# LLNL/parelagmc

Measured on AMD Instinct MI355X. Metric: MC samples/sec (SPDE field + Darcy QoI) at stated DoF; SpMV HBM GB/s vs roofline, higher is better.
Workload: dtype f64; 1 GPU; PDESampler cube_tet r=5, 595968 DoF (n_s=196608, n_u=399360, nnz(A)=4299072), 1 MC level, corlen 0.1, SPDE field only (BASELINE config 2), 4 x 64 realizations per step, all converged; tolerance=MINRES 300 / rel 1e-6 / abs 1e-12, solver=hybridization, batch=64, streams=4, parallelism=sample-farm x1, precond_storage=fp32

## Files before the change

include/pmc.h:

```cpp
#ifndef PMC_H_
#define PMC_H_

#include <stddef.h>
#include <stdint.h>

#ifdef __cplusplus
extern "C" {
#endif

#define PMC_OK 0
#define PMC_ERR_INVALID (-1)
#define PMC_ERR_DEVICE (-2)
#define PMC_ERR_COMM (-3)
#define PMC_ERR_INTERNAL (-4)

enum pmc_memspace { PMC_MEM_HOST = 0, PMC_MEM_DEVICE = 1 };
enum pmc_projection { PMC_PROJ_NONE = 0, PMC_PROJ_GATHER = 1, PMC_PROJ_L2 = 2 };
enum pmc_storage { PMC_STORAGE_FP32 = 0, PMC_STORAGE_FP64 = 1 };

typedef struct pmc_ctx pmc_ctx;
typedef struct pmc_sampler pmc_sampler;
typedef struct pmc_darcy pmc_darcy;

typedef struct pmc_csr {
// ... 3 lines not shown
    const double* vals;
} pmc_csr;

typedef struct pmc_solver_opts {
    int32_t abi_version;
    int32_t max_iter;
    double rel_tol;
    double abs_tol;
    int32_t cheb_degree_M;
    double cheb_ratio_M;
    int32_t mg_smooth_degree;
    double mg_smooth_ratio;
    int32_t mg_coarse_degree;
    double mg_coarse_ratio;
    int32_t check_every;
    int32_t use_graph;
    double schur_scale;
    int32_t mg_coarsening;
    int32_t mini_max_rows;
    int32_t two_streams;
    int32_t precond_storage;
} pmc_solver_opts;

typedef struct pmc_stats {
    int32_t iterations;
    int32_t converged;
    double initial_norm;
    double final_norm;
    double solve_ms;
    double setup_ms;
} pmc_stats;

typedef struct pmc_sampler_level {
    int32_t n_u, n_s;
    pmc_csr M;
    pmc_csr B;
    const double* w_diag;
    pmc_csr P;
} pmc_sampler_level;

typedef struct pmc_hybrid_level {
    int32_t n_lambda, n_s;
    pmc_csr H;
    pmc_csr G;
    const double* z_diag;
    const double* w_diag;
    pmc_csr P;
} pmc_hybrid_level;

typedef struct pmc_hybrid_elements {
    int32_t n_u, n_s;
    pmc_csr M_pattern;
    const int32_t* c_ptr;
    const int32_t* c_elem;
    const double* c_val;
    pmc_csr B;
    const double* w_diag;
    pmc_csr P;
} pmc_hybrid_elements;
typedef struct pmc_hybrid_system pmc_hybrid_system;

typedef struct pmc_darcy_level {
    int32_t n_u, n_p;
    pmc_csr M_pattern;
    const int32_t* c_ptr;
    const int32_t* c_elem;
    const double* c_val;
    pmc_csr B;
    const double* rhs;
    const uint8_t* ess_mask;
    const double* ess_data;
    const double* obs;
    pmc_csr P;
} pmc_darcy_level;

int pmc_version(void);
#define PMC_ABI_VERSION 3
int pmc_abi_version(void);
int pmc_krylov_z_bytes(void);
int pmc_sampler_krylov_z_bytes(const pmc_sampler* s);
int pmc_darcy_krylov_z_bytes(const pmc_darcy* d);
uint64_t pmc_kernel_launches(void);
uint64_t pmc_fused_lanczos_solves(void);
const char* pmc_last_error(void);
void pmc_solver_opts_default(pmc_solver_opts* opts);

int pmc_ctx_create(int device_id, pmc_ctx** out);
int pmc_ctx_create_abi(int device_id, int abi_version, pmc_ctx** out);
#ifndef PMC_NO_ABI_CHECK_MACRO
#define pmc_ctx_create(device_id, out) pmc_ctx_create_abi((device_id), PMC_ABI_VERSION, (out))
#endif
void pmc_ctx_destroy(pmc_ctx* ctx);
int pmc_ctx_synchronize(pmc_ctx* ctx);
void* pmc_ctx_stream(pmc_ctx* ctx);
int pmc_ctx_device(const pmc_ctx* ctx);
int pmc_timer_start(pmc_ctx* ctx);
int pmc_timer_stop(pmc_ctx* ctx, double* ms);

int pmc_malloc(pmc_ctx* ctx, size_t bytes, void** dptr);
int pmc_free(pmc_ctx* ctx, void* dptr);
int pmc_memcpy_h2d(pmc_ctx* ctx, void* dst, const void* src, size_t bytes);
int pmc_memcpy_d2h(pmc_ctx* ctx, void* dst, const void* src, size_t bytes);

int pmc_rng_seed(pmc_ctx* ctx, uint64_t seed, int nparts, int mypart);
int pmc_normal_fill(pmc_ctx* ctx, double mean, double sigma2, uint64_t first_sample_id, uint32_t stream,
                    int nbatch, int n, double* out, int memspace);

int pmc_sampler_create(pmc_ctx* ctx, int nlevels, int n_mc_levels, const pmc_sampler_level* levels,
                       double alpha, double matern_g, int lognormal, const pmc_solver_opts* opts,
                       pmc_sampler** out);
int pmc_sampler_create_hybrid(pmc_ctx* ctx, int nlevels, const pmc_hybrid_level* levels, double alpha, double matern_g,
                              int lognormal, const pmc_solver_opts* opts, pmc_sampler** out);
int pmc_sampler_is_hybrid(const pmc_sampler* s);
int pmc_hybrid_build(const pmc_hybrid_elements* level, double alpha, pmc_hybrid_system** out);
int pmc_hybrid_system_level(const pmc_hybrid_system* sys, pmc_hybrid_level* view);
void pmc_hybrid_system_destroy(pmc_hybrid_system* sys);
int pmc_sampler_create_hybrid_from_elements(pmc_ctx* ctx, int nlevels, const pmc_hybrid_elements* levels, double alpha,
                                            double matern_g, int lognormal, const pmc_solver_opts* opts, pmc_sampler** out);
typedef struct pmc_kl_level {
    int32_t n_s;
    const double* w_diag;
    pmc_csr P;
} pmc_kl_level;
int pmc_sampler_create_kl(pmc_ctx* ctx, int nlevels, const pmc_kl_level* levels, int nmodes, const double* evals,
                          const double* evect0, int lognormal, pmc_sampler** out);
int pmc_sampler_is_kl(const pmc_sampler* s);
typedef struct pmc_kl_eigs_opts {
    double tol;
    int32_t max_iter;
    int32_t guard;
    int32_t degree;
    uint64_t seed;
} pmc_kl_eigs_opts;
typedef struct pmc_kl_eigs_info {
    int32_t iterations;
    int32_t block_products;
    int32_t converged;
    double max_residual_rel;
    double gap_rel;
    double seconds;
} pmc_kl_eigs_info;
void pmc_kl_eigs_opts_default(pmc_kl_eigs_opts* opts);
int pmc_kl_matern_apply(pmc_ctx* ctx, int dim, int n, const double* centroids, const double* w_diag, double corlen,
                        int ncols, const double* X, double* Y);
int pmc_kl_matern_eigs(pmc_ctx* ctx, int dim, int n, const double* centroids, const double* w_diag, double corlen,
                       int nmodes, const pmc_kl_eigs_opts* opts , double* evals ,
                       double* evect0 , pmc_kl_eigs_info* info );
void pmc_sampler_destroy(pmc_sampler* s);
int pmc_sampler_set_projection(pmc_sampler* s, int level, int kind, const pmc_csr* Gt,
                               const int32_t* gather_idx, const double* inv_w_orig, int orig_size);
int pmc_sampler_num_levels(const pmc_sampler* s);
int pmc_sampler_xi_size(const pmc_sampler* s, int level);
int pmc_sampler_sample_size(const pmc_sampler* s, int level);
int64_t pmc_sampler_nnz(const pmc_sampler* s, int level);
int pmc_sampler_batch_width(const pmc_sampler* s, int level);
int pmc_sampler_true_p(const pmc_sampler* s, int level, pmc_csr* out);
int pmc_sampler_sample(pmc_sampler* s, int level, uint64_t first_sample_id, int nbatch, double* xi,
                       int memspace);
int pmc_sampler_eval(pmc_sampler* s, int level, int xi_level, int nbatch, const double* xi, double* s_out,
                     const double* init_s, int init_level, int use_init, double* embed_s_out, int memspace,
                     pmc_stats* stats);

typedef struct pmc_field_stats pmc_field_stats;
int pmc_field_stats_create(pmc_sampler* s, int level, const double* chi, int memspace, pmc_field_stats** out);
void pmc_field_stats_destroy(pmc_field_stats* fs);
int pmc_field_stats_reset(pmc_field_stats* fs);
// ... 95 lines not shown
```

parelagmc_amd/capi.py:

```python
from __future__ import annotations

import ctypes as C
import weakref
import os
from typing import Optional, Sequence

import numpy as np

_HERE = os.path.dirname(os.path.abspath(__file__))
LIB_PATH = os.path.join(_HERE, "lib", "libpmc.so")

PMC_MEM_HOST, PMC_MEM_DEVICE = 0, 1
PMC_PROJ_NONE, PMC_PROJ_GATHER, PMC_PROJ_L2 = 0, 1, 2


class PmcError(RuntimeError):
    def __init__(self, code, msg):
        super().__init__(f"libpmc error {code}: {msg}")
        self.code = code


class pmc_csr(C.Structure):
    _fields_ = [("nrows", C.c_int32), ("ncols", C.c_int32), ("rowptr", C.POINTER(C.c_int32)),
                ("colind", C.POINTER(C.c_int32)), ("vals", C.POINTER(C.c_double))]


class pmc_solver_opts(C.Structure):
    _fields_ = [("abi_version", C.c_int32), ("max_iter", C.c_int32), ("rel_tol", C.c_double), ("abs_tol", C.c_double),
                ("cheb_degree_M", C.c_int32), ("cheb_ratio_M", C.c_double),
                ("mg_smooth_degree", C.c_int32), ("mg_smooth_ratio", C.c_double),
                ("mg_coarse_degree", C.c_int32), ("mg_coarse_ratio", C.c_double), ("check_every", C.c_int32),
                ("use_graph", C.c_int32), ("schur_scale", C.c_double), ("mg_coarsening", C.c_int32), ("mini_max_rows", C.c_int32),
                ("two_streams", C.c_int32), ("precond_storage", C.c_int32)]


PMC_ABI_VERSION = 3
PMC_STORAGE_FP32, PMC_STORAGE_FP64 = 0, 1


class pmc_stats(C.Structure):
    _fields_ = [("iterations", C.c_int32), ("converged", C.c_int32), ("initial_norm", C.c_double),
                ("final_norm", C.c_double), ("solve_ms", C.c_double), ("setup_ms", C.c_double)]


class pmc_sampler_level(C.Structure):
    _fields_ = [("n_u", C.c_int32), ("n_s", C.c_int32), ("M", pmc_csr), ("B", pmc_csr),
                ("w_diag", C.POINTER(C.c_double)), ("P", pmc_csr)]


class pmc_hybrid_level(C.Structure):
    _fields_ = [("n_lambda", C.c_int32), ("n_s", C.c_int32), ("H", pmc_csr), ("G", pmc_csr),
                ("z_diag", C.POINTER(C.c_double)), ("w_diag", C.POINTER(C.c_double)), ("P", pmc_csr)]


class pmc_hybrid_elements(C.Structure):
    _fields_ = [("n_u", C.c_int32), ("n_s", C.c_int32), ("M_pattern", pmc_csr), ("c_ptr", C.POINTER(C.c_int32)),
                ("c_elem", C.POINTER(C.c_int32)), ("c_val", C.POINTER(C.c_double)), ("B", pmc_csr),
                ("w_diag", C.POINTER(C.c_double)), ("P", pmc_csr)]


class pmc_kl_level(C.Structure):
    _fields_ = [("n_s", C.c_int32), ("w_diag", C.POINTER(C.c_double)), ("P", pmc_csr)]


class pmc_kl_eigs_opts(C.Structure):
    _fields_ = [("tol", C.c_double), ("max_iter", C.c_int32), ("guard", C.c_int32), ("degree", C.c_int32),
                ("seed", C.c_uint64)]


class pmc_kl_eigs_info(C.Structure):
    _fields_ = [("iterations", C.c_int32), ("block_products", C.c_int32), ("converged", C.c_int32),
                ("max_residual_rel", C.c_double), ("gap_rel", C.c_double), ("seconds", C.c_double)]


class pmc_darcy_level(C.Structure):
    _fields_ = [("n_u", C.c_int32), ("n_p", C.c_int32), ("M_pattern", pmc_csr), ("c_ptr", C.POINTER(C.c_int32)),
                ("c_elem", C.POINTER(C.c_int32)), ("c_val", C.POINTER(C.c_double)), ("B", pmc_csr),
                ("rhs", C.POINTER(C.c_double)), ("ess_mask", C.POINTER(C.c_uint8)),
                ("ess_data", C.POINTER(C.c_double)), ("obs", C.POINTER(C.c_double)), ("P", pmc_csr)]


_VP = C.c_void_p
_DP = C.c_void_p
SYMBOLS = {
    "pmc_version": (C.c_int, []),
    "pmc_last_error": (C.c_char_p, []),
    "pmc_solver_opts_default": (None, [C.POINTER(pmc_solver_opts)]),
    "pmc_abi_version": (C.c_int, []),
    "pmc_krylov_z_bytes": (C.c_int, []),
    "pmc_sampler_krylov_z_bytes": (C.c_int, [_VP]),
    "pmc_darcy_krylov_z_bytes": (C.c_int, [_VP]),
    "pmc_kernel_launches": (C.c_uint64, []),
    "pmc_fused_lanczos_solves": (C.c_uint64, []),
    "pmc_ctx_create": (C.c_int, [C.c_int, C.POINTER(_VP)]),
    "pmc_ctx_create_abi": (C.c_int, [C.c_int, C.c_int, C.POINTER(_VP)]),
    "pmc_ctx_destroy": (None, [_VP]),
    "pmc_ctx_synchronize": (C.c_int, [_VP]),
    "pmc_ctx_stream": (_VP, [_VP]),
    "pmc_ctx_device": (C.c_int, [_VP]),
    "pmc_timer_start": (C.c_int, [_VP]),
    "pmc_timer_stop": (C.c_int, [_VP, C.POINTER(C.c_double)]),
    "pmc_malloc": (C.c_int, [_VP, C.c_size_t, C.POINTER(_VP)]),
    "pmc_free": (C.c_int, [_VP, _VP]),
    "pmc_memcpy_h2d": (C.c_int, [_VP, _VP, _VP, C.c_size_t]),
    "pmc_memcpy_d2h": (C.c_int, [_VP, _VP, _VP, C.c_size_t]),
    "pmc_rng_seed": (C.c_int, [_VP, C.c_uint64, C.c_int, C.c_int]),
    "pmc_normal_fill": (C.c_int, [_VP, C.c_double, C.c_double, C.c_uint64, C.c_uint32, C.c_int, C.c_int, _DP, C.c_int]),
    "pmc_sampler_create": (C.c_int, [_VP, C.c_int, C.c_int, C.POINTER(pmc_sampler_level), C.c_double, C.c_double,
                                     C.c_int, C.POINTER(pmc_solver_opts), C.POINTER(_VP)]),
    "pmc_sampler_create_hybrid": (C.c_int, [_VP, C.c_int, C.POINTER(pmc_hybrid_level), C.c_double, C.c_double, C.c_int,
                                            C.POINTER(pmc_solver_opts), C.POINTER(_VP)]),
    "pmc_sampler_is_hybrid": (C.c_int, [_VP]),
    "pmc_sampler_create_kl": (C.c_int, [_VP, C.c_int, C.POINTER(pmc_kl_level), C.c_int, C.POINTER(C.c_double),
                                        C.POINTER(C.c_double), C.c_int, C.POINTER(_VP)]),
    "pmc_sampler_is_kl": (C.c_int, [_VP]),
    "pmc_kl_eigs_opts_default": (None, [C.POINTER(pmc_kl_eigs_opts)]),
    "pmc_kl_matern_apply": (C.c_int, [_VP, C.c_int, C.c_int, C.POINTER(C.c_double), C.POINTER(C.c_double), C.c_double, C.c_int,
                                      C.POINTER(C.c_double), C.POINTER(C.c_double)]),
    "pmc_kl_matern_eigs": (C.c_int, [_VP, C.c_int, C.c_int, C.POINTER(C.c_double), C.POINTER(C.c_double), C.c_double, C.c_int,
                                     C.POINTER(pmc_kl_eigs_opts), C.POINTER(C.c_double), C.POINTER(C.c_double),
                                     C.POINTER(pmc_kl_eigs_info)]),
    "pmc_hybrid_build": (C.c_int, [C.POINTER(pmc_hybrid_elements), C.c_double, C.POINTER(_VP)]),
    "pmc_hybrid_system_level": (C.c_int, [_VP, C.POINTER(pmc_hybrid_level)]),
    "pmc_hybrid_system_destroy": (None, [_VP]),
    "pmc_sampler_create_hybrid_from_elements": (C.c_int, [_VP, C.c_int, C.POINTER(pmc_hybrid_elements), C.c_double, C.c_double,
                                                          C.c_int, C.POINTER(pmc_solver_opts), C.POINTER(_VP)]),
    "pmc_sampler_smoother_time": (C.c_int, [_VP, C.POINTER(C.c_double), C.POINTER(C.c_int64), C.POINTER(C.c_double)]),
    "pmc_sampler_smoother_bytes": (C.c_int, [_VP, C.c_int, C.c_int, C.POINTER(C.c_double)]),
    "pmc_sampler_vcycle_info": (C.c_int, [_VP, C.c_int, C.c_int, C.POINTER(C.c_int), C.POINTER(C.c_int64)]),
    "pmc_sampler_vcycle_level": (C.c_int, [_VP, C.c_int, C.c_int, C.POINTER(C.c_int), C.POINTER(C.c_double)]),
    "pmc_sampler_vcycle_prolongator": (C.c_int, [_VP, C.c_int, C.c_int, C.POINTER(C.c_int), C.POINTER(C.c_int),
                                                 C.POINTER(C.c_int64), C.POINTER(C.c_int32), C.POINTER(C.c_int32),
                                                 C.POINTER(C.c_double)]),
    "pmc_sampler_destroy": (None, [_VP]),
    "pmc_sampler_set_projection": (C.c_int, [_VP, C.c_int, C.c_int, C.POINTER(pmc_csr), C.POINTER(C.c_int32),
                                             C.POINTER(C.c_double), C.c_int]),
    "pmc_sampler_num_levels": (C.c_int, [_VP]),
    "pmc_sampler_xi_size": (C.c_int, [_VP, C.c_int]),
    "pmc_sampler_sample_size": (C.c_int, [_VP, C.c_int]),
    "pmc_sampler_batch_width": (C.c_int, [_VP, C.c_int]),
    "pmc_darcy_batch_width": (C.c_int, [_VP, C.c_int]),
    "pmc_darcy_set_operator_timing": (C.c_int, [_VP, C.c_int]),
    "pmc_darcy_operator_time": (C.c_int, [_VP, C.POINTER(C.c_double), C.POINTER(C.c_int64), C.POINTER(C.c_double)]),
    "pmc_darcy_operator_bytes": (C.c_int, [_VP, C.c_int, C.c_int, C.POINTER(C.c_double)]),
    "pmc_darcy_poly_time": (C.c_int, [_VP, C.POINTER(C.c_double), C.POINTER(C.c_int64), C.POINTER(C.c_double)]),
    "pmc_darcy_poly_bytes": (C.c_int, [_VP, C.c_int, C.c_int, C.POINTER(C.c_double)]),
    "pmc_sampler_nnz": (C.c_int64, [_VP, C.c_int]),
    "pmc_sampler_true_p": (C.c_int, [_VP, C.c_int, C.POINTER(pmc_csr)]),
    "pmc_sampler_sample": (C.c_int, [_VP, C.c_int, C.c_uint64, C.c_int, _DP, C.c_int]),
    "pmc_sampler_eval": (C.c_int, [_VP, C.c_int, C.c_int, C.c_int, _DP, _DP, _DP, C.c_int, C.c_int, _DP, C.c_int,
                                   C.POINTER(pmc_stats)]),
    "pmc_sampler_mult": (C.c_int, [_VP, C.c_int, C.c_int, _DP, _DP, C.c_int, C.c_int, C.POINTER(pmc_stats)]),
    "pmc_sampler_apply_preconditioner": (C.c_int, [_VP, C.c_int, C.c_int, _DP, _DP, C.c_int]),
    "pmc_sampler_apply_operator": (C.c_int, [_VP, C.c_int, C.c_int, _DP, _DP, C.c_int, C.c_int, C.POINTER(C.c_double),
                                             C.POINTER(C.c_double)]),
    "pmc_sampler_set_operator_timing": (C.c_int, [_VP, C.c_int]),
    "pmc_sampler_operator_time": (C.c_int, [_VP, C.POINTER(C.c_double), C.POINTER(C.c_int64)]),
    "pmc_sampler_operator_event_overhead": (C.c_int, [_VP, C.POINTER(C.c_double)]),
    "pmc_conditioner_create": (C.c_int, [_VP, C.c_int, C.POINTER(pmc_csr), C.POINTER(C.c_double), C.POINTER(C.c_double),
                                         C.POINTER(_VP)]),
    "pmc_conditioner_destroy": (None, [_VP]),
    "pmc_conditioner_num_obs": (C.c_int, [_VP]),
    "pmc_conditioner_level": (C.c_int, [_VP, C.c_int, C.POINTER(C.c_int), C.POINTER(C.c_int64), C.POINTER(C.c_double),
                                        C.POINTER(C.c_double), C.POINTER(C.c_int32), C.POINTER(C.c_int32),
                                        C.POINTER(C.c_double)]),
    "pmc_conditioner_apply": (C.c_int, [_VP, C.c_int, C.c_int, _DP, _DP, _DP, C.c_int, C.c_int]),
    "pmc_sampler_set_conditioner": (C.c_int, [_VP, _VP]),
    "pmc_field_stats_create": (C.c_int, [_VP, C.c_int, _DP, C.c_int, C.POINTER(_VP)]),
    "pmc_field_stats_destroy": (None, [_VP]),
    "pmc_field_stats_reset": (C.c_int, [_VP]),
    "pmc_field_stats_accumulate": (C.c_int, [_VP, C.c_int, _DP, C.c_int]),
    "pmc_field_stats_run": (C.c_int, [_VP, C.c_uint64, C.c_int64]),
    "pmc_field_stats_read": (C.c_int, [_VP, _DP, _DP, _DP, C.POINTER(C.c_int64), C.c_int]),
    "pmc_field_stats_read_sums": (C.c_int, [_VP, _DP, C.POINTER(C.c_int64), C.c_int]),
    "pmc_field_stats_chi_dot": (C.c_int, [_VP, C.c_int, _DP, _DP, C.c_int]),
    "pmc_sampler_l2_error": (C.c_int, [_VP, C.c_int, C.c_int, _DP, C.c_double, _DP, C.c_int]),
    "pmc_sampler_max_error": (C.c_int, [_VP, C.c_int, C.c_int, _DP, C.c_double, _DP, C.c_int]),
    "pmc_sampler_set_output_hierarchy": (C.c_int, [_VP, C.c_int, C.POINTER(pmc_csr), C.POINTER(C.c_double)]),
    "pmc_darcy_create": (C.c_int, [_VP, C.c_int, C.c_int, C.POINTER(pmc_darcy_level), C.c_int,
                                   C.POINTER(pmc_solver_opts), C.POINTER(_VP)]),
    "pmc_darcy_create_hybrid": (C.c_int, [_VP, C.c_int, C.c_int, C.POINTER(pmc_darcy_level), C.c_int,
                                          C.POINTER(pmc_solver_opts), C.POINTER(_VP)]),
    "pmc_darcy_destroy": (None, [_VP]),
    "pmc_darcy_num_dofs": (C.c_int, [_VP, C.c_int]),
    "pmc_darcy_num_pressure_dofs": (C.c_int, [_VP, C.c_int]),
    "pmc_darcy_nnz": (C.c_int64, [_VP, C.c_int]),
    "pmc_darcy_solve_fwd": (C.c_int, [_VP, C.c_int, C.c_int, _DP, C.POINTER(C.c_double), C.POINTER(C.c_double), _DP,
                                      C.c_int, C.POINTER(pmc_stats)]),
    "pmc_darcy_solve_fwd_pressure": (C.c_int, [_VP, C.c_int, C.c_int, _DP, _DP, C.POINTER(C.c_double),
                                               C.POINTER(C.c_double), C.c_int, C.c_int, C.POINTER(pmc_stats)]),
    "pmc_level_fields_create": (C.c_int, [_VP, _VP, C.c_int, C.c_int, C.POINTER(_VP)]),
    "pmc_level_fields_destroy": (None, [_VP]),
    "pmc_level_fields_reset": (C.c_int, [_VP]),
    "pmc_level_fields_accumulate": (C.c_int, [_VP, C.c_int, _DP, _DP, C.c_int]),
    "pmc_level_fields_accumulate_weighted": (C.c_int, [_VP, C.c_int, _DP, _DP, _DP, _DP, C.c_int]),
    "pmc_level_fields_read_sums": (C.c_int, [_VP, _DP, C.POINTER(C.c_int64), C.c_int]),
    "pmc_level_fields_size": (C.c_int, [_VP, C.POINTER(C.c_int), C.POINTER(C.c_int)]),
    "pmc_level_fields_parents": (C.c_int, [_VP, C.POINTER(C.c_int32)]),
    "pmc_darcy_apply_preconditioner": (C.c_int, [_VP, C.c_int, C.c_int, _DP, _DP, _DP, C.c_int]),
    "pmc_darcy_apply_operator": (C.c_int, [_VP, C.c_int, C.c_int, _DP, _DP, _DP, C.c_int]),
    "pmc_darcy_vcycle_level": (C.c_int, [_VP, C.c_int, C.c_int, C.POINTER(C.c_int), C.POINTER(C.c_double)]),
    "pmc_darcy_vcycle_prolongator": (C.c_int, [_VP, C.c_int, C.c_int, C.POINTER(C.c_int), C.POINTER(C.c_int),
                                               C.POINTER(C.c_int64), C.POINTER(C.c_int32), C.POINTER(C.c_int32),
                                               C.POINTER(C.c_double)]),
    "pmc_darcy_set_observations": (C.c_int, [_VP, C.c_int, C.POINTER(pmc_csr)]),
    "pmc_darcy_num_observations": (C.c_int, [_VP, C.c_int]),
    "pmc_darcy_compute_G": (C.c_int, [_VP, C.c_int, C.c_int, _DP, C.POINTER(C.c_double), C.POINTER(C.c_double),
                                      C.POINTER(C.c_double), C.c_int, C.POINTER(pmc_stats)]),
    "pmc_comm_unique_id": (C.c_int, [_VP]),
    "pmc_comm_init": (C.c_int, [_VP, _VP, C.c_int, C.c_int]),
    "pmc_comm_destroy": (C.c_int, [_VP]),
    "pmc_allreduce_sum_f64": (C.c_int, [_VP, C.POINTER(C.c_double), C.c_int]),
}

_lib = None


def load_library(path: Optional[str] = None):
    global _lib
    if _lib is not None and path is None:
        return _lib
    p = path or os.environ.get("PMC_LIB") or LIB_PATH
    if not os.path.exists(p):
        raise PmcError(-2, f"{p} not found - build it with `make` / __graft_entry__.build() (no CPU fallback)")
    lib = C.CDLL(p)
    for name, (res, args) in SYMBOLS.items():
        fn = getattr(lib, name)
        fn.restype = res
        fn.argtypes = args
    if path is None:
        _lib = lib
    return lib


def _check(rc):
    if rc != 0:
        raise PmcError(rc, load_library().pmc_last_error().decode("utf-8", "replace"))


def _i32(a):
    return np.ascontiguousarray(a, dtype=np.int32)


def _f64(a):
    return np.ascontiguousarray(a, dtype=np.float64)


def _ptr(a, ctype):
    return a.ctypes.data_as(C.POINTER(ctype))


class _Keep:

    def __init__(self):
        self.refs = []

    def csr(self, m) -> pmc_csr:
        if m is None:
            return pmc_csr(0, 0, None, None, None)
        m = m.tocsr()
        rp, ci, v = _i32(m.indptr), _i32(m.indices), _f64(m.data)
        self.refs += [rp, ci, v]
        return pmc_csr(m.shape[0], m.shape[1], _ptr(rp, C.c_int32), _ptr(ci, C.c_int32), _ptr(v, C.c_double))

    def f64(self, a):
        a = _f64(a)
        self.refs.append(a)
        return _ptr(a, C.c_double)

    def i32(self, a):
        a = _i32(a)
        self.refs.append(a)
        return _ptr(a, C.c_int32)

    def u8(self, a):
        a = np.ascontiguousarray(a, dtype=np.uint8)
        self.refs.append(a)
        return _ptr(a, C.c_uint8)


def hybrid_build(pattern, c_ptr, c_elem, c_val, B, w_diag, alpha, P=None):
    import scipy.sparse as sp
    lib = load_library()
    keep = _Keep()
    n_s, n_u = B.shape
    lv = pmc_hybrid_elements(n_u, n_s, keep.csr(pattern), keep.i32(c_ptr), keep.i32(c_elem), keep.f64(c_val), keep.csr(B),
                             keep.f64(w_diag), keep.csr(P))
    h = _VP()
    _check(lib.pmc_hybrid_build(C.byref(lv), float(alpha), C.byref(h)))
    try:
        v = pmc_hybrid_level()
        _check(lib.pmc_hybrid_system_level(h, C.byref(v)))

        def mat(c):
            rp = np.ctypeslib.as_array(c.rowptr, (c.nrows + 1,)).copy()
            nnz = int(rp[-1])
            return sp.csr_matrix((np.ctypeslib.as_array(c.vals, (nnz,)).copy(), np.ctypeslib.as_array(c.colind, (nnz,)).copy(), rp),
                                 shape=(c.nrows, c.ncols))
        return mat(v.H), mat(v.G), np.ctypeslib.as_array(v.z_diag, (n_s,)).copy()
    finally:
        lib.pmc_hybrid_system_destroy(h)


def library_hybrid_builder(space, alpha):
    from .fe.rt0 import mass_contributions
    pat, c_ptr, c_elem, c_val = mass_contributions(space.emass)
    return hybrid_build(pat, c_ptr, c_elem, c_val, space.B, space.vol, alpha)


# ... 828 lines not shown
```

parelagmc_amd/csrc/capi.hip:

```cpp
#include <dlfcn.h>

#include <atomic>
#include <cstdlib>
#include <cstring>
#include <mutex>

#include "handles.hpp"

namespace pmc {

static thread_local std::string g_last_error;
void set_last_error(const std::string& m) { g_last_error = m; }

void Ctx::activate() const { PMC_HIP(hipSetDevice(device)); }
void Ctx::phase_mark(int i) const { PMC_HIP(hipEventRecord(ev_phase[i], stream)); }
void Ctx::phase_report(pmc_stats* stats, int nb) const {
    PMC_HIP(hipEventSynchronize(ev_phase[2]));
    float setup = 0.f, solve = 0.f;
    PMC_HIP(hipEventElapsedTime(&setup, ev_phase[0], ev_phase[1]));
    PMC_HIP(hipEventElapsedTime(&solve, ev_phase[1], ev_phase[2]));
    for (int k = 0; k < nb; ++k) {
        stats[k].setup_ms = (double)setup / nb;
        stats[k].solve_ms = (double)solve / nb;
    }
}

static std::atomic<int> g_live_ctx[64];
int Ctx::contexts_on_device(int device) { return g_live_ctx[device & 63].load(); }

Lanes Ctx::lanes(bool split) {
    if (split && !stream2) {
        PMC_HIP(hipStreamCreateWithFlags(&stream2, hipStreamNonBlocking));
        PMC_HIP(hipEventCreateWithFlags(&ev_fork, hipEventDisableTiming));
        PMC_HIP(hipEventCreateWithFlags(&ev_join, hipEventDisableTiming));
    }
    return Lanes{stream, split ? stream2 : stream, ev_fork, ev_join, split};
}

template <class F>
static int guarded(F&& f) {
    try {
        f();
        return PMC_OK;
    } catch (const Error& e) {
        set_last_error(e.what());
        return e.code;
    } catch (const std::bad_alloc&) {
        set_last_error("host allocation failed");
        return PMC_ERR_INTERNAL;
    } catch (const std::exception& e) {
        set_last_error(e.what());
        return PMC_ERR_INTERNAL;
    } catch (...) {
        set_last_error("unknown exception");
        return PMC_ERR_INTERNAL;
    }
}

struct UniqueId { char internal[128]; };
struct Rccl {
    void* lib = nullptr;
    int (*GetUniqueId)(UniqueId*) = nullptr;
    int (*CommInitRank)(void**, int, UniqueId, int) = nullptr;
    int (*AllReduce)(const void*, void*, size_t, int, int, void*, hipStream_t) = nullptr;
    int (*CommDestroy)(void*) = nullptr;
    const char* (*GetErrorString)(int) = nullptr;
};
static Rccl& rccl() {
    static Rccl r;
    static std::once_flag once;
    std::call_once(once, [] {
        const char* names[] = {"librccl.so.1", "librccl.so", "/opt/rocm/lib/librccl.so.1", "/opt/rocm/lib/librccl.so"};
        for (const char* n : names) {
            r.lib = dlopen(n, RTLD_NOW | RTLD_LOCAL);
            if (r.lib) break;
        }
        if (!r.lib) return;
        r.GetUniqueId = reinterpret_cast<decltype(r.GetUniqueId)>(dlsym(r.lib, "ncclGetUniqueId"));
        r.CommInitRank = reinterpret_cast<decltype(r.CommInitRank)>(dlsym(r.lib, "ncclCommInitRank"));
        r.AllReduce = reinterpret_cast<decltype(r.AllReduce)>(dlsym(r.lib, "ncclAllReduce"));
        r.CommDestroy = reinterpret_cast<decltype(r.CommDestroy)>(dlsym(r.lib, "ncclCommDestroy"));
        r.GetErrorString = reinterpret_cast<decltype(r.GetErrorString)>(dlsym(r.lib, "ncclGetErrorString"));
    });
    if (!r.lib || !r.GetUniqueId || !r.CommInitRank || !r.AllReduce || !r.CommDestroy)
        throw Error(PMC_ERR_COMM, "RCCL (librccl.so) could not be loaded");
    return r;
}
static void rccl_check(int rc, const char* what) {
    if (rc != 0) {
        Rccl& r = rccl();
        throw Error(PMC_ERR_COMM, std::string(what) + ": " + (r.GetErrorString ? r.GetErrorString(rc) : "RCCL error"));
    }
}

}

using namespace pmc;

extern "C" {

int pmc_version(void) { return 100; }
int pmc_abi_version(void) { return PMC_ABI_VERSION; }
int pmc_krylov_z_bytes(void) { return 4; }
uint64_t pmc_kernel_launches(void) { return kernel_launch_count(); }
uint64_t pmc_fused_lanczos_solves(void) { return fused_lanczos_solve_count(); }
const char* pmc_last_error(void) { return g_last_error.c_str(); }

static void check_abi(const pmc_solver_opts& o) {
    if (o.abi_version != PMC_ABI_VERSION)
        throw Error(PMC_ERR_INVALID, "pmc_solver_opts.abi_version is " + std::to_string(o.abi_version) + ", this library has " +
                                         std::to_string(PMC_ABI_VERSION) +
                                         ": fill the struct with pmc_solver_opts_default() of the header you compile against");
}

void pmc_solver_opts_default(pmc_solver_opts* o) {
    if (!o) return;
    o->max_iter = 300;
    o->rel_tol = 1e-6;
    o->abs_tol = 1e-12;
    o->abi_version = PMC_ABI_VERSION;
    o->cheb_degree_M = 0;
    o->cheb_ratio_M = 0.0;
    o->mg_smooth_degree = 2;
    o->mg_smooth_ratio = 8.0;
    o->mg_coarse_degree = 12;
    o->mg_coarse_ratio = 100.0;
    o->check_every = 2;
    o->schur_scale = 1.0;
    o->mg_coarsening = 2;
    o->mini_max_rows = 6000;
    o->two_streams = 0;
    o->use_graph = 0;
    o->precond_storage = PMC_STORAGE_FP32;
}

#undef pmc_ctx_create
int pmc_ctx_create(int device_id, pmc_ctx** out);
int pmc_ctx_create_abi(int device_id, int abi_version, pmc_ctx** out) {
    if (abi_version != PMC_ABI_VERSION) {
        if (out) *out = nullptr;
        set_last_error("caller was compiled against PMC_ABI_VERSION " + std::to_string(abi_version) + ", this library has " +
                       std::to_string(PMC_ABI_VERSION) + " (layout of pmc_solver_opts / pmc_stats): rebuild against include/pmc.h");
        return PMC_ERR_INVALID;
    }
    return pmc_ctx_create(device_id, out);
}
int pmc_ctx_create(int device_id, pmc_ctx** out) {
    return guarded([&] {
        PMC_REQUIRE(out != nullptr, "pmc_ctx_create: out is NULL");
        *out = nullptr;
        int ndev = 0;
        hipError_t e = hipGetDeviceCount(&ndev);
        if (e != hipSuccess || ndev == 0)
            throw Error(PMC_ERR_DEVICE, "no HIP device available (libpmc has no CPU fallback)");
        PMC_REQUIRE(device_id >= 0 && device_id < ndev, "pmc_ctx_create: device id out of range");
        std::unique_ptr<pmc_ctx> c(new pmc_ctx());
        c->device = device_id;
        PMC_HIP(hipSetDevice(device_id));
        PMC_HIP(hipStreamCreateWithFlags(&c->stream, hipStreamNonBlocking));
        PMC_HIP(hipEventCreate(&c->ev0));
        PMC_HIP(hipEventCreate(&c->ev1));
        for (hipEvent_t& e : c->ev_phase) PMC_HIP(hipEventCreate(&e));
        PMC_HIP(hipHostMalloc(reinterpret_cast<void**>(&c->h_flag), sizeof(int) * 16, hipHostMallocDefault));
        PMC_HIP(hipHostMalloc(reinterpret_cast<void**>(&c->h_scal), sizeof(double) * pmc::Ctx::kHostScratch, hipHostMallocDefault));
        g_live_ctx[device_id & 63].fetch_add(1);
        *out = c.release();
    });
}

void pmc_ctx_destroy(pmc_ctx* c) {
    if (!c) return;
    g_live_ctx[c->device & 63].fetch_sub(1);
    (void)hipSetDevice(c->device);
    if (c->nccl) {
        try { rccl().CommDestroy(c->nccl); } catch (...) {}
        c->nccl = nullptr;
    }
    if (c->stream) (void)hipStreamSynchronize(c->stream);
    if (c->stream2) (void)hipStreamSynchronize(c->stream2);
    if (c->h_flag) (void)hipHostFree(c->h_flag);
    if (c->h_scal) (void)hipHostFree(c->h_scal);
    if (c->ev0) (void)hipEventDestroy(c->ev0);
    if (c->ev1) (void)hipEventDestroy(c->ev1);
    for (hipEvent_t e : c->ev_phase)
        if (e) (void)hipEventDestroy(e);
    for (hipEvent_t e : {c->ev_fork, c->ev_join})
        if (e) (void)hipEventDestroy(e);
    if (c->stream2) (void)hipStreamDestroy(c->stream2);
// ... 724 lines not shown
```

parelagmc_amd/csrc/handles.hpp:

```cpp
#pragma once
#include "solver.hpp"

namespace pmc {

HostCsr schur_host(const HostCsr& B, const HostCsr& Bt, const std::vector<double>& dM, const double* diag_add);
std::unique_ptr<Multigrid> build_sa_chain(const HostCsr& K, const std::vector<double>& w, const pmc_solver_opts& o,
                                          hipStream_t st);

bool spd_dense_inverse(const HostCsr& S, std::vector<double>& inv);

struct Conditioner;

struct SamplerLevel {
    double ratio_M = 8.0;
    int n_u = 0, n_s = 0;
    int64_t nnz = 0;
    Sell A;
    Sell M;
    DevBuf<double> dinvM;
    DevBuf<double> M_scaled;
    DevBuf<double> w_sqrt;
    int proj = PMC_PROJ_NONE;
    int out_size = 0;
    Sell Gt;
    DevBuf<int> gather;
    DevBuf<double> inv_w;
    HostCsr P_host;
    Sell Gz;
    Sell Gl;
    Sell Ptz;
    DevBuf<double> zw_sqrt;
    DevBuf<int> lam_new2old, lam_old2new;
    std::vector<int> lam_n2o_host;
};

struct Sampler {
    Ctx& ctx;
    int nlevels, n_mc;
    double alpha, g;
    bool lognormal;
    pmc_solver_opts opts;
    std::vector<SamplerLevel> lv;
    Multigrid mg;
    std::vector<std::unique_ptr<Multigrid>> amg;
    double anisotropy = 1.0;
    bool hybrid = false;
    bool kl = false;
    int kl_m = 0;
    std::vector<DevBuf<double>> kl_phi;
    Conditioner* cond = nullptr;
    std::vector<double> w0_host;
    std::vector<HostCsr> out_P;
    std::vector<double> out_w0;
    struct ErrChain {
        std::vector<int> nrows, ncols;
        std::vector<DevBuf<int>> rp, ci;
        std::vector<DevBuf<double>> v;
        DevBuf<double> w0;
        bool ready = false;
        void upload(const std::vector<const HostCsr*>& P, const std::vector<double>& w, hipStream_t st);
    };
    ErrChain err_own, err_out;
    OpTimer vc_timer;
    MinresWork work;
    DevBuf<double> rhs, sol, tA, tB, cx, cd, cx2, stage_in, stage_out, stage_emb, mini_scratch;
    DevBuf<pmc_stats> mini_stats;

    Sampler(Ctx& c, int nlevels, int n_mc, const pmc_sampler_level* in, double alpha, double g, bool lognormal,
            const pmc_solver_opts& o);
    Sampler(Ctx& c, int nlevels, const pmc_hybrid_level* in, double alpha, double g, bool lognormal, const pmc_solver_opts& o);
    Sampler(Ctx& c, int nlevels, const pmc_kl_level* in, int nmodes, const double* evals, const double* evect0, bool lognormal);
    double smoother_bytes(int level, int nb) const;
    void vcycle_level(int level, int vlevel, int* nvlevels, double* info) const;
    const HostCsr& vcycle_prolongator(int level, int vlevel, HostCsr& scratch) const;
    size_t system_rows(int level) const { return hybrid ? (size_t)lv[level].n_u : (size_t)lv[level].n_u + lv[level].n_s; }
    void set_projection(int level, int kind, const pmc_csr* Gt, const int32_t* idx, const double* inv_w, int orig_size);
    void sample(int level, uint64_t first_id, int nbatch, double* xi, int memspace);
    void eval(int level, int xi_level, int nbatch, const double* xi, double* s_out, const double* init_s, int init_level,
              bool use_init, double* emb_out, int memspace, pmc_stats* stats);
    void apply_operator(int level, int nb, const double* x, double* y, int memspace, int repeat, double* avg_ms,
                        double* bytes);
    void mult(int level, int nbatch, const double* rhs, double* sol, bool use_guess, int memspace, pmc_stats* stats);
    void apply_preconditioner(int level, int nbatch, const double* r, double* z, int memspace);

    void set_output_hierarchy(int nlev, const pmc_csr* P_orig, const double* w0_orig);
    void field_error(int level, int nbatch, const double* coeff, double exact, double* err, int memspace, bool max_err);
    int launch_width(int level) const;

  private:
    void ensure(int level, int nb);
    void solve_system(int level, int nb, bool zero_guess, int x_row0, int x_nrows, pmc_stats* stats);
    PrecFn preconditioner(int level, int nb, int degM, Multigrid* mgp, int mg_l0);
    void eval_chunk(int level, int xi_level, int nb, const double* xi_d, double* s_d, const double* init_d,
                    int init_level, bool use_init, double* emb_d, pmc_stats* stats);
    void eval_kl(int level, int xi_level, int nbatch, const double* xi, double* s_out, double* emb_out, int memspace,
                 pmc_stats* stats);
};

constexpr int kCondMaxObs = 512;
struct Conditioner {
    Sampler& smp;
    int nobs, mp;
    bool noisy = false;
    struct Level {
        int n = 0, ld = 0;
        HostCsr H;
        DevBuf<int> hrp, hci;
        DevBuf<double> hv, K, Ainv;
        std::vector<double> A;
    };
    std::vector<Level> lv;
    DevBuf<double> y, sqrt_sigma2, coef, stage_g, stage_z;
    Conditioner(Sampler& s, int nobs, const pmc_csr* H0, const double* y, const double* sigma2);
    ~Conditioner() { if (smp.cond == this) smp.cond = nullptr; }
    void apply(int level, int nbatch, const double* g, const double* zeta, double* out, bool apply_exp, int memspace);
    void apply_device(int level, int nbatch, const double* g_d, const double* zeta_d, double* out_d, bool apply_exp);
    void export_level(int level, int* n, int64_t* nnz, double* K, double* A, int32_t* rowptr, int32_t* colind,
                      double* vals) const;

  private:
    void build_K_solves(int level);
    void build_K_kl(int level);
};

struct FieldStats {
    Sampler& smp;
    int level, n;
    bool has_chi;
    int64_t count = 0;
    DevBuf<double> chi, acc, dots, part, xi, sbuf;
    FieldStats(Sampler& s, int level, const double* chi, int memspace);
    void reset();
    void accumulate(int nbatch, const double* s, int memspace);
    void run(uint64_t first_id, int64_t nsamples);
    void read(double* expectation, double* second_moment, double* chi_cov, int64_t* count, int memspace);
    void read_sums(double* sums, int64_t* count, int memspace);
    void chi_dots(int nbatch, const double* s, double* out, int memspace);

  private:
    void check_size() const;
    void accumulate_device(int nbatch, const double* s_d);
};

struct Darcy;
struct LevelFields {
    Ctx& ctx;
    int level, n, nc;
    bool coupled;
    int64_t count = 0;
    std::vector<int> parent_host;
    DevBuf<int> parent;
    DevBuf<double> acc, pbuf, cbuf;
    LevelFields(Ctx& c, const Darcy& d, int level, bool coupled);
    void reset();
    void accumulate(int nbatch, const double* p_fine, const double* p_coarse, int memspace);
    void accumulate_weighted(int nbatch, const double* p_fine, const double* w_fine, const double* p_coarse,
                             const double* w_coarse, int memspace);
    void read_sums(double* sums, int64_t* count, int memspace);

  private:
    void accumulate_device(int nbatch, const double* pf, const double* pc);
    void accumulate_weighted_device(int nbatch, const double* pf, const double* wf, const double* pc, const double* wc);
};

void kl_matern_apply(pmc_ctx* c, int dim, int n, const double* centroids, const double* w_diag, double corlen, int ncols,
                     const double* X, double* Y);
void kl_matern_eigs(pmc_ctx* c, int dim, int n, const double* centroids, const double* w_diag, double corlen, int nmodes,
                    const pmc_kl_eigs_opts* opts, double* evals, double* evect0, pmc_kl_eigs_info* info);

void kl_eval(hipStream_t st, int n, int m, int nb, const double* phi, const double* xi, int n_xi, double* s, double* emb,
             bool lognormal);

struct DarcyLevel {
    int n_u = 0, n_p = 0, n_coef = 0;
// ... 108 lines not shown
```

parelagmc_amd/csrc/kernels.hip:

```cpp
#include "sell_rows.hpp"

#include <cstddef>
#include <cstdlib>

#include <algorithm>
#include <atomic>

namespace pmc {

static unsigned dot_grid_bound();
int dot_capacity(int nrows, int nb) {
    const size_t slice_blocks = ((size_t)nrows + 63) / 64 / (kBlock / kWave) + 1;
    const size_t flat_blocks = ((size_t)nrows * nb / (nb >= 32 ? 4 : (nb >= 2 ? 2 : 1)) + kBlock - 1) / kBlock;
    const size_t bounded = std::min<size_t>(std::max(slice_blocks, flat_blocks), dot_grid_bound());
    return (int)std::max<size_t>(bounded, 256 + slice_blocks) + 2;
}

template <int NB, int BV, typename XT = double>
__device__ __forceinline__ void sell_row_product(const int* __restrict__ slice_off, const int* __restrict__ cols,
                                                 const double* __restrict__ vals, const XT* __restrict__ x,
                                                 int slice, int lane, int LD, double (&acc)[Lay<NB>::T][Lay<NB>::C]) {
    const int off = slice_off[slice];
    const int width = (slice_off[slice + 1] - off) >> 6;
    sell_row_range<NB, BV, false, true, false, XT>(cols, vals, x, nullptr, off, width, lane, LD, acc);
}

template <int NB, int BV, int MODE, bool DOT, int TAG, bool NT = false, bool R8 = false, bool DL = false, typename XT = double,
          typename YT = double, int LZ = 0>
__global__ __launch_bounds__(kBlock, (NB >= 32 && BV == 0 && sizeof(XT) == 4 ? 3 : 1)) void sell_spmm_kernel(int nrows, int nslices, const int* __restrict__ slice_off,
                                                           const int* __restrict__ sched,
                                                           const int* __restrict__ cols,
                                                           const double* __restrict__ vals,
                                                           const XT* __restrict__ x, typename ident<YT>::type* __restrict__ y,
                                                           const double* __restrict__ r,
                                                           const typename ident<XT>::type* __restrict__ dot_with,
                                                           double* __restrict__ partial, int ld,
                                                           k::LanczosUpdate lz = k::LanczosUpdate{}) {
    static_assert(!R8 || (MODE == 2 && !DOT), "fused restriction goes with the residual");
    static_assert(LZ == 0 || (BV == 0 && MODE == 0 && !R8 && sizeof(YT) == 8 && DOT == (LZ == 1)),
                  "Lanczos passes: shared values, plain product; the dot-only pass has the dot, the update passes none");
    static_assert(sizeof(YT) == 8 || (MODE == 0 && !DOT && !NT), "fp32 result: plain products only");
    const int LD = row_ld<NB>(ld);
    {
        const int c0 = col0<NB>();
        x += c0;
        if constexpr (LZ != 1) y += c0;
        if constexpr (BV) vals = shift_bv<BV>(vals, c0);
        if constexpr (MODE == 2) r += c0;
        if constexpr (DOT && !DL) dot_with += c0;
        if constexpr (DOT || R8) partial += c0;
        if constexpr (LZ >= 2) {
            lz.v1 += c0; lz.y32 += c0;
            lz.c0 += c0; lz.c1 += c0; lz.c2 += c0;
        }
    }
    static_assert(!DL || (DOT && !BV && Lay<NB>::T > 1), "diagonal-last serves the fused <x, Ax> of shared-value operators");
    constexpr int C = Lay<NB>::C, T = Lay<NB>::T, G = Lay<NB>::G;
    const int lane = threadIdx.x & (kWave - 1);
    const int g = lane / T, t = lane % T;
    double p[C];
#pragma unroll
    for (int c = 0; c < C; ++c) p[c] = 0.0;
    const SliceWalk sw = slice_walk(nslices);
    for (int si = sw.begin; si < sw.end; si += sw.stride) {
        const int slice = sched ? sched[si] : si;
        double acc[T][C];
        constexpr bool LEAN_DL = DL && lean_range<NB>();
        double xd[DL && !LEAN_DL ? T : 1][C];
        if constexpr (LEAN_DL) {
            const int off = slice_off[slice];
            sell_row_range<NB, false, false, true, NT, XT>(cols, vals, x, nullptr, off, (slice_off[slice + 1] - off) >> 6,
                                                             lane, LD, acc, nullptr, p);
        } else if constexpr (DL) {
            const int off = slice_off[slice];
            sell_row_range<NB, false, false, true, NT, XT>(cols, vals, x, nullptr, off, (slice_off[slice + 1] - off) >> 6,
                                                             lane, LD, acc, xd);
        } else if constexpr (NT) {
            const int off = slice_off[slice];
            sell_row_range<NB, BV, false, true, true, XT>(cols, vals, x, nullptr, off, (slice_off[slice + 1] - off) >> 6, lane, LD, acc);
        } else {
            sell_row_product<NB, BV, XT>(slice_off, cols, vals, x, slice, lane, LD, acc);
        }
#pragma unroll
        for (int rs = 0; rs < T; ++rs) {
            const int row = slice * kWave + rs * G + g;
            if (row < nrows) {
                const size_t at = (size_t)row * LD + t * C;
                if constexpr (MODE == 1) {
                    double old[C];
                    load_c<C>(y + at, old);
#pragma unroll
                    for (int c = 0; c < C; ++c) acc[rs][c] += old[c];
                } else if constexpr (MODE == 2) {
                    double rv[C];
                    load_c<C>(r + at, rv);
#pragma unroll
                    for (int c = 0; c < C; ++c) acc[rs][c] = rv[c] - acc[rs][c];
                }
                if constexpr (LZ >= 2) {
                    double bv[C], yv[C];
                    load_c_nt<NT, C>(lz.v1 + at, bv);
                    if constexpr (LZ == 2) {
                        load_c_nt<NT, C>(y + at, yv);
                    } else {
#pragma unroll
                        for (int c = 0; c < C; ++c) yv[c] = 0.0;
                    }
                    lanczos_combine<C>(lz.c0, lz.c1, lz.c2, t * C, acc[rs], bv, yv);
                    store_c<C>(y + at, yv);
                    store_v<C>(lz.y32 + at, yv);
                } else if constexpr (LZ == 1) {
                } else if constexpr (sizeof(YT) == 8) store_c_stream<NT, C>(y + at, acc[rs]);
                else store_v<C>(y + at, acc[rs]);
                if constexpr (LEAN_DL) {
                } else if constexpr (DL) {
#pragma unroll
                    for (int c = 0; c < C; ++c) p[c] = fma(xd[rs][c], acc[rs][c], p[c]);
                } else if constexpr (DOT) {
                    double w[C];
                    load_v<C>(dot_with + at, w);
#pragma unroll
                    for (int c = 0; c < C; ++c) p[c] = fma(w[c], acc[rs][c], p[c]);
                }
            } else if constexpr (R8) {
#pragma unroll
                for (int c = 0; c < C; ++c) acc[rs][c] = 0.0;
            }
            if constexpr (R8) {
                double s[C];
#pragma unroll
                for (int c = 0; c < C; ++c) {
                    double v = acc[rs][c];
                    v += __shfl_xor(v, T, kWave);
                    v += __shfl_xor(v, 2 * T, kWave);
                    v += __shfl_xor(v, 4 * T, kWave);
                    s[c] = v;
                }
                if ((g & 7) == 0 && row < nrows) store_c<C>(partial + (size_t)(row >> 3) * LD + t * C, s);
            }
        }
    }
    if constexpr (DOT) reduce_cols_store<NB>(p, partial, LD);
}

template <int NB, int BV, bool DOT, typename OT = double>
__global__ __launch_bounds__(kBlock) void sell_cheb_kernel(int nrows, int nslices, const int* __restrict__ slice_off,
                                                           const int* __restrict__ sched,
                                                           const int* __restrict__ cols,
                                                           const double* __restrict__ vals,
                                                           const double* __restrict__ dinv,
                                                           const double* __restrict__ r,
                                                           const double* __restrict__ xin, double* __restrict__ d,
                                                           OT* __restrict__ xout, double a, double b,
                                                           double* __restrict__ partial, int ld) {
    constexpr int C = Lay<NB>::C, T = Lay<NB>::T, G = Lay<NB>::G;
    const int LD = row_ld<NB>(ld);
    {
        const int c0 = col0<NB>();
        r += c0; xin += c0; d += c0; xout += c0;
        if constexpr (BV) { vals = shift_bv<BV>(vals, c0); dinv += c0; }
        if constexpr (DOT) partial += c0;
    }
    const int lane = threadIdx.x & (kWave - 1);
    const int g = lane / T, t = lane % T;
    double p[C];
#pragma unroll
    for (int c = 0; c < C; ++c) p[c] = 0.0;
    const SliceWalk sw = slice_walk(nslices);
    for (int si = sw.begin; si < sw.end; si += sw.stride) {
        const int slice = sched ? sched[si] : si;
        double acc[T][C];
        sell_row_product<NB, BV>(slice_off, cols, vals, xin, slice, lane, LD, acc);
#pragma unroll
        for (int rs = 0; rs < T; ++rs) {
            const int row = slice * kWave + rs * G + g;
            if (row >= nrows) continue;
            const size_t at = (size_t)row * LD + t * C;
            double rv[C], dv[C], xv[C], di[C];
            load_c<C>(r + at, rv);
            load_c<C>(xin + at, xv);
            if (a != 0.0) {
                load_c<C>(d + at, dv);
// ... 682 lines not shown
#pragma unroll
    for (int c = 0; c < C; ++c) p[c] = 0.0;
    for (size_t i = (size_t)blockIdx.x * kBlock + threadIdx.x; i < nflat; i += (size_t)gridDim.x * kBlock) {
        double v[C];
        load_c<C>(in + i * C, v);
        round_to<OT>(v);
        if constexpr (DOT) {
            double rv[C];
            load_c<C>(r + i * C, rv);
#pragma unroll
            for (int c = 0; c < C; ++c) p[c] = fma(rv[c], v[c], p[c]);
        }
        store_v<C>(out + i * C, v);
    }
    if constexpr (DOT) reduce_flat_store<NB>(p, partial, row_ld<NB>(ld));
}

template <int NB>
__global__ __launch_bounds__(kBlock) void copy_r32_kernel(size_t nflat, const double* __restrict__ in,
                                                          double* __restrict__ out, float* __restrict__ out32) {
    constexpr int C = Lay<NB>::C;
    for (size_t i = (size_t)blockIdx.x * kBlock + threadIdx.x; i < nflat; i += (size_t)gridDim.x * kBlock) {
        double v[C];
        load_c<C>(in + i * C, v);
        store_c<C>(out + i * C, v);
        store_v<C>(out32 + i * C, v);
    }
}

template <int NB, bool NT = false>
__global__ __launch_bounds__(kBlock) void lincomb3_kernel(size_t nflat, const double* __restrict__ c0,
                                                          const double* __restrict__ a, const double* __restrict__ c1,
                                                          const double* __restrict__ b, const double* __restrict__ c2,
                                                          double* __restrict__ y, int ld, float* __restrict__ y32 = nullptr) {
    constexpr int C = Lay<NB>::C;
    const size_t i = (size_t)blockIdx.x * kBlock + threadIdx.x;
    if (i >= nflat) return;
    const size_t e = i * C;
    const int k0 = (int)(e % row_ld<NB>(ld));
    double av[C], bv[C], yv[C];
    load_c_nt<NT, C>(a + e, av);
    load_c_nt<NT, C>(b + e, bv);
    load_c_nt<NT, C>(y + e, yv);
    lanczos_combine<C>(c0, c1, c2, k0, av, bv, yv);
    store_c<C>(y + e, yv);
    if (y32) store_v<C>(y32 + e, yv);
}

template <int NB, bool NT, typename UT>
__global__ __launch_bounds__(kBlock) void minres_wx_kernel(size_t nflat, const double* __restrict__ c0,
                                                           const UT* __restrict__ u, const double* __restrict__ c1,
                                                           double* __restrict__ w0, const double* __restrict__ c2,
                                                           const double* __restrict__ w1, const double* __restrict__ c3,
                                                           double* __restrict__ x, int ld) {
    constexpr int C = Lay<NB>::C;
    const size_t i = (size_t)blockIdx.x * kBlock + threadIdx.x;
    if (i >= nflat) return;
    const size_t e = i * C;
    const int k0 = (int)(e % row_ld<NB>(ld));
    double uv[C], w0v[C], w1v[C], xv[C];
    load_v_nt<NT, C>(u + e, uv);
    load_c_nt<NT, C>(w0 + e, w0v);
    load_c_nt<NT, C>(w1 + e, w1v);
    load_c_nt<NT, C>(x + e, xv);
#pragma unroll
    for (int c = 0; c < C; ++c) {
        w0v[c] = c0[k0 + c] * uv[c] + c1[k0 + c] * w0v[c] + c2[k0 + c] * w1v[c];
        xv[c] += c3[k0 + c] * w0v[c];
    }
    store_c_nt<NT, C>(w0 + e, w0v);
    store_c_nt<NT, C>(x + e, xv);
}

template <bool NT, typename UT, int C>
__device__ __forceinline__ void load_raw_nt(const UT* __restrict__ p, RawVec<UT, C>& r) {
    if constexpr (NT) {
#pragma unroll
        for (int i = 0; i < C; ++i) r.v[i] = __builtin_nontemporal_load(p + i);
    } else {
        load_raw<C>(p, r);
    }
}

template <int NB, bool NT, typename UT>
__global__ __launch_bounds__(kBlock) void minres_wx_deferred_kernel(size_t nflat, k::WxDeferred B,
                                                                    const double* __restrict__ cW, double* __restrict__ w0,
                                                                    double* __restrict__ w1, double* __restrict__ x, int ld) {
    constexpr int C = Lay<NB>::C;
    const size_t i = (size_t)blockIdx.x * kBlock + threadIdx.x;
    if (i >= nflat) return;
    const size_t e = i * C;
    const int k0 = (int)(e % row_ld<NB>(ld));
    double a[C], b[C], xv[C];
    if (B.first) {
#pragma unroll
        for (int c = 0; c < C; ++c) a[c] = b[c] = 0.0;
    } else {
        load_c_nt<NT, C>(w0 + e, a);
        load_c_nt<NT, C>(w1 + e, b);
    }
    if (B.first && B.x_zero) {
#pragma unroll
        for (int c = 0; c < C; ++c) xv[c] = 0.0;
    } else {
        load_c_nt<NT, C>(x + e, xv);
    }
    for (int t = 0; t < B.cnt; t += k::kWxDefer) {
        RawVec<UT, C> uv[k::kWxDefer];
#pragma unroll
        for (int j = 0; j < k::kWxDefer; ++j)
            if (t + j < B.cnt) load_raw_nt<NT>(static_cast<const UT*>(B.u[t + j]) + e, uv[j]);
#pragma unroll
        for (int j = 0; j < k::kWxDefer; ++j) {
            if (t + j < B.cnt) {
                const double* cj = cW + (size_t)B.slot[t + j] * 4 * kMaxBatch + k0;
#pragma unroll
                for (int c = 0; c < C; ++c) {
                    const double wn = cj[c] * (double)uv[j].v[c] + cj[kMaxBatch + c] * a[c] + cj[2 * kMaxBatch + c] * b[c];
                    xv[c] += cj[3 * kMaxBatch + c] * wn;
                    a[c] = b[c];
                    b[c] = wn;
                }
            }
        }
    }
    if (!B.last) {
        store_c_nt<NT, C>(w0 + e, a);
        store_c_nt<NT, C>(w1 + e, b);
    }
    store_c_nt<NT, C>(x + e, xv);
}

template <int NB>
__global__ __launch_bounds__(kBlock) void wdot_kernel(size_t nflat, const double* __restrict__ w,
                                                      const double* __restrict__ x, double* __restrict__ partial, int ld) {
    constexpr int C = Lay<NB>::C;
    const int W = row_ld<NB>(ld);
    double p[C];
#pragma unroll
    for (int c = 0; c < C; ++c) p[c] = 0.0;
    for (size_t i = (size_t)blockIdx.x * kBlock + threadIdx.x; i < nflat; i += (size_t)gridDim.x * kBlock) {
        double xv[C];
        load_c<C>(x + i * C, xv);
        const double ww = w[(i * C) / W];
#pragma unroll
        for (int c = 0; c < C; ++c) p[c] = fma(ww, xv[c], p[c]);
    }
    reduce_flat_store<NB>(p, partial, W);
}

__global__ void fill_kernel(size_t n, double* __restrict__ x, double v) {
    size_t i = (size_t)blockIdx.x * blockDim.x + threadIdx.x;
    const size_t stride = (size_t)gridDim.x * blockDim.x;
    for (; i < n; i += stride) x[i] = v;
}

static constexpr int kScalBlock = 1024;
__device__ __forceinline__ double reduce_partials(const double* __restrict__ partial, int nblocks, int nb,
                                                  const double* __restrict__ partial2 = nullptr, int nblocks2 = 0) {
    __shared__ double lds[kScalBlock];
    const int k = threadIdx.x % nb, q = threadIdx.x / nb, nq = kScalBlock / nb;
    double s0 = 0.0, s1 = 0.0, s2 = 0.0, s3 = 0.0, s4 = 0.0, s5 = 0.0, s6 = 0.0, s7 = 0.0;
    int b = q;
    for (; b + 7 * nq < nblocks; b += 8 * nq) {
        s0 += partial[(size_t)b * nb + k];
        s1 += partial[(size_t)(b + nq) * nb + k];
        s2 += partial[(size_t)(b + 2 * nq) * nb + k];
        s3 += partial[(size_t)(b + 3 * nq) * nb + k];
        s4 += partial[(size_t)(b + 4 * nq) * nb + k];
        s5 += partial[(size_t)(b + 5 * nq) * nb + k];
        s6 += partial[(size_t)(b + 6 * nq) * nb + k];
        s7 += partial[(size_t)(b + 7 * nq) * nb + k];
    }
    for (; b < nblocks; b += nq) s0 += partial[(size_t)b * nb + k];
    for (b = q; b + 3 * nq < nblocks2; b += 4 * nq) {
        s4 += partial2[(size_t)b * nb + k];
        s5 += partial2[(size_t)(b + nq) * nb + k];
        s6 += partial2[(size_t)(b + 2 * nq) * nb + k];
        s7 += partial2[(size_t)(b + 3 * nq) * nb + k];
    }
    for (; b < nblocks2; b += nq) s1 += partial2[(size_t)b * nb + k];
    s0 += s4;
    s1 += s5;
    s2 += s6;
    s3 += s7;
    const double s = (s0 + s1) + (s2 + s3);
    __syncthreads();
    lds[threadIdx.x] = s;
    __syncthreads();
    int groups = nq;
    for (int stride = nq >> 1; stride >= 32; stride >>= 1) {
        if (q < stride) lds[threadIdx.x] += lds[threadIdx.x + stride * nb];
        __syncthreads();
        groups = stride;
    }
    double t = 0.0;
    if ((int)threadIdx.x < nb)
        for (int g = 0; g < groups; ++g) t += lds[g * nb + threadIdx.x];
    return t;
}

__device__ __forceinline__ void count_active(k::MinresState* st, int nb, bool bump) {
    __syncthreads();
    const int na = __syncthreads_count((int)threadIdx.x < nb && st->active[threadIdx.x] != 0);
    if (threadIdx.x == 0) {
        st->n_active = na;
        st->it = bump ? st->it + 1 : 0;
    }
}

__global__ __launch_bounds__(kScalBlock) void minres_init_kernel(k::MinresState* st, const double* __restrict__ partial,
                                                             int nblocks, int nb, double rel_tol, double abs_tol,
                                                             const double* __restrict__ partial2, int nblocks2, int ring) {
// ... 801 lines not shown
        const double d1 = block_sum(p, red);
        const double ib = 1.0 / beta;
        const double alpha = d1 * ib * ib;
        const double cV0 = ib, cV1 = -alpha * ib, cV2 = -beta / beta_old;
        const double delta = gamma1 * alpha - gamma0 * sigma1 * beta;
        const double rho3 = sigma0 * beta;
        const double rho2 = sigma1 * alpha + gamma0 * gamma1 * beta;
        for (int i = tid; i < n; i += kTailThreads) v0[i] = cV0 * q[i] + cV1 * v1[i] + cV2 * v0[i];
        __syncthreads();
        const double d2 = prec(v0, u0);
        if (d2 < 0.0 || d2 != d2) flag = -1;
        const double beta_new = d2 > 0.0 ? sqrt(d2) : 0.0;
        const double rho1 = hypot(delta, beta_new);
        const double ir = rho1 > 0.0 ? 1.0 / rho1 : 0.0;
        const double cW0 = ir / beta, cW1 = -rho3 * ir, cW2 = -rho2 * ir;
        gamma0 = gamma1;
        gamma1 = delta * ir;
        const double cW3 = gamma1 * eta;
        sigma0 = sigma1;
        sigma1 = beta_new * ir;
        eta = -sigma1 * eta;
        beta_old = beta;
        beta = beta_new;
        for (int i = tid; i < P.x_nrows; i += kTailThreads) {
            const double w = cW0 * u1[P.x_row0 + i] + cW1 * w0[i] + cW2 * w1[i];
            w0[i] = w;
            xs[i] += cW3 * w;
        }
        ++it;
        if (fabs(eta) <= goal || beta_new == 0.0 || flag != 0) active = false;
        double* t;
        t = u0; u0 = u1; u1 = t;
        t = v0; v0 = v1; v1 = t;
        t = w0; w0 = w1; w1 = t;
        __syncthreads();
    }
    for (int i = tid; i < P.x_nrows; i += kTailThreads) x[(size_t)(P.x_row0 + i) * nb + k] = xs[i];
    if (tid == 0) {
        stats[k].iterations = it;
        stats[k].converged = flag != 0 ? -1 : (fabs(eta) <= goal ? 1 : 0);
        stats[k].initial_norm = eta0;
        stats[k].final_norm = fabs(eta);
        stats[k].solve_ms = 0.0;
        stats[k].setup_ms = 0.0;
    }
}

#define PMC_DISPATCH_NB(nb, ...)                                          \
    switch (nb) {                                                         \
        case 1: { constexpr int NB = 1; __VA_ARGS__; } break;             \
        case 2: { constexpr int NB = 2; __VA_ARGS__; } break;             \
        case 4: { constexpr int NB = 4; __VA_ARGS__; } break;             \
        case 8: { constexpr int NB = 8; __VA_ARGS__; } break;             \
        case 16: { constexpr int NB = 16; __VA_ARGS__; } break;           \
        case 32: case 64: case 128: case 256: { constexpr int NB = 32; __VA_ARGS__; } break;    \
        default: throw Error(PMC_ERR_INTERNAL, "unsupported batch width"); \
    }

#define PMC_DISPATCH_NARROW(nb, ...)                                      \
    switch (nb) {                                                         \
        case 1: { constexpr int NB = 1; __VA_ARGS__; } break;             \
        case 2: { constexpr int NB = 2; __VA_ARGS__; } break;             \
        case 4: { constexpr int NB = 4; __VA_ARGS__; } break;             \
        case 8: { constexpr int NB = 8; __VA_ARGS__; } break;             \
        default: throw Error(PMC_ERR_INTERNAL, "row-split level kernels serve launches of 1, 2, 4 or 8 realizations"); \
    }

static inline dim3 groups(dim3 g, int nb) { return dim3(g.x, nb > kGroup ? (unsigned)(nb / kGroup) : 1u); }
static inline bool xcd_layout(dim3 g, int nb) {
    static const bool on = [] { const char* e = lab_env("PMC_XCD_GROUPS"); return e && atoi(e) != 0; }();
    return on && nb > kGroup && g.x >= 16;
}
static inline dim3 groups_xcd(dim3 g, int nb) {
    if (!xcd_layout(g, nb)) return groups(g, nb);
    return dim3(8u, (unsigned)(nb / kGroup), (g.x + 7u) / 8u);
}
static inline int dot_blocks(dim3 g, int nb) { return xcd_layout(g, nb) ? (int)((g.x + 7u) / 8u * 8u) : (int)g.x; }
static inline dim3 groups(unsigned g, int nb) { return groups(dim3(g), nb); }
static inline dim3 groups(int g, int nb) { return groups(dim3((unsigned)g), nb); }
static inline dim3 grid_rows(int n) { return dim3((unsigned)((n + kBlock - 1) / kBlock)); }
static inline dim3 grid_slices(int nslices) { return dim3((unsigned)((nslices + kBlock / kWave - 1) / (kBlock / kWave))); }
static inline int lay_c(int nb) { return nb >= 32 ? 4 : (nb >= 2 ? 2 : 1); }
static inline size_t flat_count(int n, int nb) { return (size_t)n * nb / lay_c(nb); }
static inline dim3 grid_flat(int n, int nb) { return dim3((unsigned)((flat_count(n, nb) + kBlock - 1) / kBlock)); }
static std::atomic<uint64_t> g_kernel_launches{0};
uint64_t kernel_launch_count() { return g_kernel_launches.load(std::memory_order_relaxed); }
void count_kernel_launches(int n) { g_kernel_launches.fetch_add((uint64_t)n, std::memory_order_relaxed); }
static inline void check_launch(int n = 1) {
    PMC_HIP(hipGetLastError());
    count_kernel_launches(n);
}
static inline void check_offsets32(const SellView& A, int nb) {
    if ((uint64_t)std::max(A.nrows, A.ncols_hint) * (uint64_t)nb >= (1ull << 32))
        throw Error(PMC_ERR_INVALID, "operand exceeds the 32-bit gather offsets of the SpMM kernels (rows x batch width >= 2^32)");
}
static inline bool nt_flat(size_t doubles) {
    static const double limit = [] {
        const char* e = lab_env("PMC_NT_FLAT_MB");
        return (e ? atof(e) : 8.0) * 1024.0 * 1024.0;
    }();
    return limit > 0.0 && (double)doubles * 8.0 > limit;
}

static unsigned dot_grid_bound() {
    static const unsigned v = [] {
        const char* e = lab_env("PMC_DOT_GRID");
        const long x = e ? atol(e) : 0;
        return x >= 8 ? (unsigned)x : 4096u;
    }();
    return v;
}

namespace k {

static inline dim3 grid_bounded(dim3 g, bool bounded) { return bounded ? dim3(std::min(g.x, dot_grid_bound())) : g; }

static inline bool nt_streams(const SellView& A, int nb, bool in_loop) {
    const double bytes = 12.0 * (double)A.nslices * 64.0 * 6.0 + 16.0 * nb * (double)A.nrows;
    static const double loop_limit = [] {
        const char* e = lab_env("PMC_NT_MIN_MB");
        return (e ? atof(e) : 128.0) * 1024.0 * 1024.0;
    }();
    return bytes > (in_loop ? loop_limit : 256.0 * 1024.0 * 1024.0);
}

static inline bool nt_poly(const SellView& A, int nb) {
    static const double limit = [] {
        const char* e = lab_env("PMC_NT_POLY_MB");
        return (e ? atof(e) : 32.0) * 1024.0 * 1024.0;
    }();
    const double bytes = 12.0 * (double)A.nslices * 64.0 * 6.0 + 16.0 * nb * (double)A.nrows;
    return limit > 0.0 && bytes > limit;
}

#define PMC_SPMM_LZ(NTF, DLF, LZF)                                                                                          \
    sell_spmm_kernel<NB, false, 0, (LZF) == 1, TAG, NTF, false, DLF, XT, double, LZF><<<groups_xcd(g, nb), kBlock, 0, st>>>( \
        A.nrows, A.nslices, A.slice_off, A.sched, A.cols, A.vals, x, y, nullptr, dot_with, dot_partial, nb, *lz)

template <int NB, int TAG, typename XT>
static void spmm_launch(hipStream_t st, int nb, dim3 g, const SellView& A, const XT* x, double* y, bool accumulate,
                        double* dot_partial, const XT* dot_with, int lz_mode = 0, const LanczosUpdate* lz = nullptr) {
    const bool dl = TAG == 1 && Lay<NB>::T > 1 && A.diag_last && dot_with == x;
    if constexpr (!std::is_same<XT, double>::value) {
        if (A.bv || accumulate) throw Error(PMC_ERR_INTERNAL, "spmm: fp32 input with per-realization values / accumulation");
        if constexpr (TAG == 1) {
            if (lz_mode) {
                const bool ntl = nt_streams(A, NB, true);
                constexpr bool kDl = Lay<NB>::T > 1;
                if (lz_mode == 1) {
                    if (ntl) { if (dl) PMC_SPMM_LZ(true, kDl, 1); else PMC_SPMM_LZ(true, false, 1); }
                    else { if (dl) PMC_SPMM_LZ(false, kDl, 1); else PMC_SPMM_LZ(false, false, 1); }
                } else if (lz_mode == 2) {
                    if (ntl) PMC_SPMM_LZ(true, false, 2); else PMC_SPMM_LZ(false, false, 2);
                } else {
                    if (ntl) PMC_SPMM_LZ(true, false, 3); else PMC_SPMM_LZ(false, false, 3);
                }
                return;
            }
        }
        const bool nt = TAG != 0 && nt_streams(A, NB, dot_partial != nullptr);
        if (nt) {
            if (dot_partial && dl)
                sell_spmm_kernel<NB, false, 0, true, TAG, true, false, (Lay<NB>::T > 1), XT><<<groups_xcd(g, nb), kBlock, 0, st>>>(A.nrows, A.nslices, A.slice_off, A.sched, A.cols, A.vals, x, y, nullptr, dot_with, dot_partial, nb);
            else if (dot_partial)
                sell_spmm_kernel<NB, false, 0, true, TAG, true, false, false, XT><<<groups_xcd(g, nb), kBlock, 0, st>>>(A.nrows, A.nslices, A.slice_off, A.sched, A.cols, A.vals, x, y, nullptr, dot_with, dot_partial, nb);
            else
// ... 31 lines not shown
            sell_spmm_kernel<NB, false, 1, false, TAG, true><<<groups_xcd(g, nb), kBlock, 0, st>>>(A.nrows, A.nslices, A.slice_off, A.sched, A.cols, A.vals, x, y, nullptr, nullptr, nullptr, nb);
        else
            sell_spmm_kernel<NB, false, 0, false, TAG, true><<<groups_xcd(g, nb), kBlock, 0, st>>>(A.nrows, A.nslices, A.slice_off, A.sched, A.cols, A.vals, x, y, nullptr, nullptr, nullptr, nb);
    } else {
        if (dot_partial && dl)
            sell_spmm_kernel<NB, false, 0, true, TAG, false, false, (Lay<NB>::T > 1)><<<groups_xcd(g, nb), kBlock, 0, st>>>(A.nrows, A.nslices, A.slice_off, A.sched, A.cols, A.vals, x, y, nullptr, dot_with, dot_partial, nb);
        else if (dot_partial)
            sell_spmm_kernel<NB, false, 0, true, TAG><<<groups_xcd(g, nb), kBlock, 0, st>>>(A.nrows, A.nslices, A.slice_off, A.sched, A.cols, A.vals, x, y, nullptr, dot_with, dot_partial, nb);
        else if (accumulate)
            sell_spmm_kernel<NB, false, 1, false, TAG><<<groups_xcd(g, nb), kBlock, 0, st>>>(A.nrows, A.nslices, A.slice_off, A.sched, A.cols, A.vals, x, y, nullptr, nullptr, nullptr, nb);
        else
            sell_spmm_kernel<NB, false, 0, false, TAG><<<groups_xcd(g, nb), kBlock, 0, st>>>(A.nrows, A.nslices, A.slice_off, A.sched, A.cols, A.vals, x, y, nullptr, nullptr, nullptr, nb);
    }
}

template <typename XT>
static int spmm_t(hipStream_t st, int nb, const SellView& A, const XT* x, double* y, bool accumulate, double* dot_partial,
                  const XT* dot_with, int lz_mode = 0, const LanczosUpdate* lz = nullptr) {
    check_offsets32(A, nb);
    if (A.nrows == 0) return 0;
    if (dot_partial && !dot_with) throw Error(PMC_ERR_INTERNAL, "spmm: fused dot without its second vector");
    dim3 g = grid_bounded(grid_slices(A.nslices), dot_partial != nullptr);
    const bool two_stage = dot_partial && A.tag != 0 && !A.bv && grid_slices(A.nslices).x > g.x;
    double* kernel_partial = dot_partial;
    if (two_stage) {
        g = grid_slices(A.nslices);
        kernel_partial = dot_partial + (size_t)kCompressBlocks * nb;
    }
    PMC_DISPATCH_NB(nb, {
        if (A.tag == 1) spmm_launch<NB, 1, XT>(st, nb, g, A, x, y, accumulate, kernel_partial, dot_with, lz_mode, lz);
        else if (A.tag == 2) spmm_launch<NB, 2, XT>(st, nb, g, A, x, y, accumulate, kernel_partial, dot_with);
        else spmm_launch<NB, 0, XT>(st, nb, g, A, x, y, accumulate, kernel_partial, dot_with);
    });
    check_launch();
    if (two_stage) {
        compress_partials_kernel<<<kCompressBlocks, 256, 0, st>>>(kernel_partial, dot_blocks(g, nb), nb, dot_partial);
        check_launch();
        return kCompressBlocks;
    }
    return dot_partial ? dot_blocks(g, nb) : 0;
}
int spmm(hipStream_t st, int nb, const SellView& A, const double* x, double* y, bool accumulate, double* dot_partial,
         const double* dot_with) {
    return spmm_t<double>(st, nb, A, x, y, accumulate, dot_partial, dot_with);
}
int spmm_z(hipStream_t st, int nb, const SellView& A, zvec x, double* y, double* dot_partial, zvec dot_with) {
    if (x.f32) return spmm_t<float>(st, nb, A, x.as<float>(), y, false, dot_partial, dot_with.as<float>());
    return spmm_t<double>(st, nb, A, x.as<double>(), y, false, dot_partial, dot_with.as<double>());
}

static void check_lanczos_pass(const SellView& A, zvec x) {
    if (!x.f32 || A.bv || A.tag != 1)
        throw Error(PMC_ERR_INTERNAL, "Lanczos operator passes: shared values, fp32-stored input, the solver's operator");
}
int spmm_z_dot(hipStream_t st, int nb, const SellView& A, zvec x, double* dot_partial) {
    check_lanczos_pass(A, x);
    const LanczosUpdate none{};
    return spmm_t<float>(st, nb, A, x.as<float>(), nullptr, false, dot_partial, x.as<float>(), 1, &none);
}
void spmm_z_update(hipStream_t st, int nb, const SellView& A, zvec x, const LanczosUpdate& lz, double* v, bool v_zero) {
    check_lanczos_pass(A, x);
    if (!lz.c0 || !lz.c1 || !lz.c2 || !lz.v1 || !lz.y32 || !v)
        throw Error(PMC_ERR_INTERNAL, "Lanczos update pass: operand missing");
    spmm_t<float>(st, nb, A, x.as<float>(), v, false, nullptr, nullptr, v_zero ? 3 : 2, &lz);
}

void residual_restrict8(hipStream_t st, int nb, const SellView& A, const double* r, const double* x, double* out,
                        double* coarse) {
    check_offsets32(A, nb);
    if (A.nrows == 0) return;
    if (A.nrows % 8 != 0) throw Error(PMC_ERR_INTERNAL, "residual_restrict8: rows are not groups of 8");
    const dim3 g = grid_slices(A.nslices);
    PMC_DISPATCH_NB(nb, {
        if (A.bv && A.f32)
            sell_spmm_kernel<NB, 2, 2, false, 0, false, true><<<groups_xcd(g, nb), kBlock, 0, st>>>(A.nrows, A.nslices, A.slice_off, A.sched, A.cols, A.vals, x, out, r, nullptr, coarse, nb);
        else if (A.bv)
            sell_spmm_kernel<NB, true, 2, false, 0, false, true><<<groups_xcd(g, nb), kBlock, 0, st>>>(A.nrows, A.nslices, A.slice_off, A.sched, A.cols, A.vals, x, out, r, nullptr, coarse, nb);
        else
            sell_spmm_kernel<NB, false, 2, false, 0, false, true><<<groups_xcd(g, nb), kBlock, 0, st>>>(A.nrows, A.nslices, A.slice_off, A.sched, A.cols, A.vals, x, out, r, nullptr, coarse, nb);
    });
    check_launch();
}

void residual(hipStream_t st, int nb, const SellView& A, const double* r, const double* x, double* out) {
    check_offsets32(A, nb);
    if (A.nrows == 0) return;
    const dim3 g = grid_slices(A.nslices);
    PMC_DISPATCH_NB(nb, {
        if (A.bv && A.f32)
            sell_spmm_kernel<NB, 2, 2, false, 0><<<groups_xcd(g, nb), kBlock, 0, st>>>(A.nrows, A.nslices, A.slice_off, A.sched, A.cols, A.vals, x, out, r, nullptr, nullptr, nb);
        else if (A.bv)
            sell_spmm_kernel<NB, true, 2, false, 0><<<groups_xcd(g, nb), kBlock, 0, st>>>(A.nrows, A.nslices, A.slice_off, A.sched, A.cols, A.vals, x, out, r, nullptr, nullptr, nb);
        else
            sell_spmm_kernel<NB, false, 2, false, 0><<<groups_xcd(g, nb), kBlock, 0, st>>>(A.nrows, A.nslices, A.slice_off, A.sched, A.cols, A.vals, x, out, r, nullptr, nullptr, nb);
    });
    check_launch();
}

template <typename OT>
static int cheb_step_t(hipStream_t st, int nb, const SellView& A, const double* dinv, bool dinv_bv, const double* r,
                       const double* xin, double* d, OT* xout, double a, double b, double* dot_partial) {
    check_offsets32(A, nb);
    if (A.nrows == 0) return 0;
    if (A.bv != dinv_bv) throw Error(PMC_ERR_INTERNAL, "cheb_step: value/diagonal batching mismatch");
    const dim3 g = grid_bounded(grid_slices(A.nslices), dot_partial != nullptr);
    PMC_DISPATCH_NB(nb, {
        if (A.bv && A.f32) {
            if (dot_partial)
                sell_cheb_kernel<NB, 2, true, OT><<<groups_xcd(g, nb), kBlock, 0, st>>>(A.nrows, A.nslices, A.slice_off, A.sched, A.cols, A.vals, dinv, r, xin, d, xout, a, b, dot_partial, nb);
            else
                sell_cheb_kernel<NB, 2, false, OT><<<groups_xcd(g, nb), kBlock, 0, st>>>(A.nrows, A.nslices, A.slice_off, A.sched, A.cols, A.vals, dinv, r, xin, d, xout, a, b, nullptr, nb);
        } else if (A.bv) {
            if (dot_partial)
                sell_cheb_kernel<NB, 1, true, OT><<<groups_xcd(g, nb), kBlock, 0, st>>>(A.nrows, A.nslices, A.slice_off, A.sched, A.cols, A.vals, dinv, r, xin, d, xout, a, b, dot_partial, nb);
            else
                sell_cheb_kernel<NB, 1, false, OT><<<groups_xcd(g, nb), kBlock, 0, st>>>(A.nrows, A.nslices, A.slice_off, A.sched, A.cols, A.vals, dinv, r, xin, d, xout, a, b, nullptr, nb);
        } else {
            if (dot_partial)
                sell_cheb_kernel<NB, 0, true, OT><<<groups_xcd(g, nb), kBlock, 0, st>>>(A.nrows, A.nslices, A.slice_off, A.sched, A.cols, A.vals, dinv, r, xin, d, xout, a, b, dot_partial, nb);
            else
                sell_cheb_kernel<NB, 0, false, OT><<<groups_xcd(g, nb), kBlock, 0, st>>>(A.nrows, A.nslices, A.slice_off, A.sched, A.cols, A.vals, dinv, r, xin, d, xout, a, b, nullptr, nb);
        }
    });
    check_launch();
    return dot_partial ? dot_blocks(g, nb) : 0;
}

int cheb_step(hipStream_t st, int nb, const SellView& A, const double* dinv, bool dinv_bv, const double* r,
              const double* xin, double* d, double* xout, double a, double b, double* dot_partial) {
    return cheb_step_t<double>(st, nb, A, dinv, dinv_bv, r, xin, d, xout, a, b, dot_partial);
}

int cheb_step_z(hipStream_t st, int nb, const SellView& A, const double* dinv, bool dinv_bv, const double* r,
                const double* xin, double* d, zvec zout, double a, double b, double* dot_partial) {
    if (zout.f32) return cheb_step_t<float>(st, nb, A, dinv, dinv_bv, r, xin, d, zout.as<float>(), a, b, dot_partial);
    return cheb_step_t<double>(st, nb, A, dinv, dinv_bv, r, xin, d, zout.as<double>(), a, b, dot_partial);
}

template <typename OT>
static int poly2_t(hipStream_t st, int nb, const SellView& As, const double* dinv, bool dinv_bv, const double* r, OT* xout,
                   double c0, double c1, double* dot_partial, const double* xadd, const double* dot_with, const int* padd_idx,
                   const double* padd_x) {
    check_offsets32(As, nb);
    if (As.nrows == 0) return 0;
    if (As.bv != dinv_bv) throw Error(PMC_ERR_INTERNAL, "poly2: value/diagonal batching mismatch");
    const dim3 g = grid_bounded(grid_slices(As.nslices), dot_partial != nullptr);
    PMC_DISPATCH_NB(nb, {
        if (As.bv && As.f32) {
            if (dot_partial)
                sell_poly2_kernel<NB, 2, true, false, OT><<<groups_xcd(g, nb), kBlock, 0, st>>>(As.nrows, As.nslices, As.slice_off, As.sched, As.cols, As.vals, dinv, r, xout, c0, c1, dot_partial, xadd, dot_with, padd_idx, padd_x, nb);
            else
                sell_poly2_kernel<NB, 2, false, false, OT><<<groups_xcd(g, nb), kBlock, 0, st>>>(As.nrows, As.nslices, As.slice_off, As.sched, As.cols, As.vals, dinv, r, xout, c0, c1, nullptr, xadd, dot_with, padd_idx, padd_x, nb);
        } else if (As.bv) {
            if (dot_partial)
                sell_poly2_kernel<NB, 1, true, false, OT><<<groups_xcd(g, nb), kBlock, 0, st>>>(As.nrows, As.nslices, As.slice_off, As.sched, As.cols, As.vals, dinv, r, xout, c0, c1, dot_partial, xadd, dot_with, padd_idx, padd_x, nb);
            else
                sell_poly2_kernel<NB, 1, false, false, OT><<<groups_xcd(g, nb), kBlock, 0, st>>>(As.nrows, As.nslices, As.slice_off, As.sched, As.cols, As.vals, dinv, r, xout, c0, c1, nullptr, xadd, dot_with, padd_idx, padd_x, nb);
        } else if (nt_poly(As, NB)) {
            if (dot_partial)
                sell_poly2_kernel<NB, 0, true, true, OT><<<groups_xcd(g, nb), kBlock, 0, st>>>(As.nrows, As.nslices, As.slice_off, As.sched, As.cols, As.vals, dinv, r, xout, c0, c1, dot_partial, xadd, dot_with, padd_idx, padd_x, nb);
            else
                sell_poly2_kernel<NB, 0, false, true, OT><<<groups_xcd(g, nb), kBlock, 0, st>>>(As.nrows, As.nslices, As.slice_off, As.sched, As.cols, As.vals, dinv, r, xout, c0, c1, nullptr, xadd, dot_with, padd_idx, padd_x, nb);
        } else {
            if (dot_partial)
                sell_poly2_kernel<NB, 0, true, false, OT><<<groups_xcd(g, nb), kBlock, 0, st>>>(As.nrows, As.nslices, As.slice_off, As.sched, As.cols, As.vals, dinv, r, xout, c0, c1, dot_partial, xadd, dot_with, padd_idx, padd_x, nb);
            else
// ... 413 lines not shown
    check_launch();
    return dot_partial ? (int)g.x : 0;
}

static inline dim3 grid_dot(int n, int nb) { return dim3(std::min(grid_flat(n, nb).x, 1024u)); }

int dot_z(hipStream_t st, int nb, int n, const double* a, zvec b, double* partial) {
    const dim3 g = grid_dot(n, nb);
    PMC_DISPATCH_NB(nb, {
        if (b.f32) dot_kernel<NB, float><<<g, kBlock, 0, st>>>(flat_count(n, nb), a, b.as<float>(), partial, nb);
        else dot_kernel<NB, double><<<g, kBlock, 0, st>>>(flat_count(n, nb), a, b.as<double>(), partial, nb);
    });
    check_launch();
    return (int)g.x;
}

int convert_z(hipStream_t st, int nb, int n, const double* in, zvec out, const double* r, double* dot_partial) {
    if (n == 0) return 0;
    const dim3 g = grid_dot(n, nb);
    PMC_DISPATCH_NB(nb, {
        if (out.f32) {
            if (dot_partial) convert_dot_kernel<NB, true, float><<<g, kBlock, 0, st>>>(flat_count(n, nb), in, out.as<float>(), r, dot_partial, nb);
            else convert_dot_kernel<NB, false, float><<<g, kBlock, 0, st>>>(flat_count(n, nb), in, out.as<float>(), nullptr, nullptr, nb);
        } else {
            if (dot_partial) convert_dot_kernel<NB, true, double><<<g, kBlock, 0, st>>>(flat_count(n, nb), in, out.as<double>(), r, dot_partial, nb);
            else convert_dot_kernel<NB, false, double><<<g, kBlock, 0, st>>>(flat_count(n, nb), in, out.as<double>(), nullptr, nullptr, nb);
        }
    });
    check_launch();
    return dot_partial ? (int)g.x : 0;
}

void copy_r32(hipStream_t st, int nb, int n, const double* in, double* out, float* out32) {
    if (n == 0) return;
    PMC_DISPATCH_NB(nb, { copy_r32_kernel<NB><<<grid_dot(n, nb), kBlock, 0, st>>>(flat_count(n, nb), in, out, out32); });
    check_launch();
}

int wdot(hipStream_t st, int nb, int n, const double* w, const double* x, double* partial) {
    const dim3 g = grid_dot(n, nb);
    PMC_DISPATCH_NB(nb, { wdot_kernel<NB><<<g, kBlock, 0, st>>>(flat_count(n, nb), w, x, partial, nb); });
    check_launch();
    return (int)g.x;
}

void reduce_final(hipStream_t st, int nb, int nblocks, const double* partial, double* out) {
    reduce_final_kernel<<<1, kScalBlock, 0, st>>>(partial, nblocks, nb, out);
    check_launch();
}

void lincomb3(hipStream_t st, int nb, int n, const double* c0, const double* a, const double* c1, const double* b,
              const double* c2, double* y, float* y32) {
    static const bool nt_on = [] { const char* e = lab_env("PMC_NT_LINCOMB"); return !e || atoi(e) != 0; }();
    const bool nt = nt_on && nt_flat((size_t)n * nb);
    PMC_DISPATCH_NB(nb, {
        if (nt) lincomb3_kernel<NB, true><<<grid_flat(n, nb), kBlock, 0, st>>>(flat_count(n, nb), c0, a, c1, b, c2, y, nb, y32);
        else lincomb3_kernel<NB><<<grid_flat(n, nb), kBlock, 0, st>>>(flat_count(n, nb), c0, a, c1, b, c2, y, nb, y32);
    });
    check_launch();
}

template <typename UT>
static void minres_wx_t(hipStream_t st, int nb, int n, const double* c0, const UT* u, const double* c1, double* w0,
                        const double* c2, const double* w1, const double* c3, double* x) {
    const bool nt = nt_flat((size_t)n * nb);
    PMC_DISPATCH_NB(nb, {
        if (nt) minres_wx_kernel<NB, true, UT><<<grid_flat(n, nb), kBlock, 0, st>>>(flat_count(n, nb), c0, u, c1, w0, c2, w1, c3, x, nb);
        else minres_wx_kernel<NB, false, UT><<<grid_flat(n, nb), kBlock, 0, st>>>(flat_count(n, nb), c0, u, c1, w0, c2, w1, c3, x, nb);
    });
}
void minres_wx(hipStream_t st, int nb, int n, const double* c0, zvec u, const double* c1, double* w0,
               const double* c2, const double* w1, const double* c3, double* x) {
    if (u.f32) minres_wx_t<float>(st, nb, n, c0, u.as<float>(), c1, w0, c2, w1, c3, x);
    else minres_wx_t<double>(st, nb, n, c0, u.as<double>(), c1, w0, c2, w1, c3, x);
    check_launch();
}

void minres_wx_deferred(hipStream_t st, int nb, int n, const MinresState* s, const WxDeferred& B, double* w0, double* w1,
                        double* x) {
    if (n == 0 || B.cnt == 0) return;
    if (B.cnt < 0 || B.cnt > kWxWindow) throw Error(PMC_ERR_INTERNAL, "minres_wx_deferred: bad count");
    const double* cW = reinterpret_cast<const double*>(reinterpret_cast<const char*>(s) + offsetof(MinresState, cW));
    const bool nt = nt_flat((size_t)n * nb);
    PMC_DISPATCH_NB(nb, {
        if (B.f32) {
            if (nt) minres_wx_deferred_kernel<NB, true, float><<<grid_flat(n, nb), kBlock, 0, st>>>(flat_count(n, nb), B, cW, w0, w1, x, nb);
            else minres_wx_deferred_kernel<NB, false, float><<<grid_flat(n, nb), kBlock, 0, st>>>(flat_count(n, nb), B, cW, w0, w1, x, nb);
        } else {
            if (nt) minres_wx_deferred_kernel<NB, true, double><<<grid_flat(n, nb), kBlock, 0, st>>>(flat_count(n, nb), B, cW, w0, w1, x, nb);
            else minres_wx_deferred_kernel<NB, false, double><<<grid_flat(n, nb), kBlock, 0, st>>>(flat_count(n, nb), B, cW, w0, w1, x, nb);
        }
    });
    check_launch();
}

void fill(hipStream_t st, size_t n, double* x, double v) {
    if (n == 0) return;
    if (v == 0.0) {
        PMC_HIP(hipMemsetAsync(x, 0, n * sizeof(double), st));
        return;
    }
    const unsigned g = (unsigned)std::min<size_t>((n + kBlock - 1) / kBlock, 2048);
    fill_kernel<<<g, kBlock, 0, st>>>(n, x, v);
    check_launch();
}

__global__ __launch_bounds__(kBlock) void scale_kernel(size_t n, const double* __restrict__ in, double a, double* __restrict__ out) {
    for (size_t i = (size_t)blockIdx.x * kBlock + threadIdx.x; i < n; i += (size_t)gridDim.x * kBlock) out[i] = a * in[i];
}
void scale(hipStream_t st, size_t n, const double* in, double a, double* out) {
    if (n == 0) return;
    const unsigned g = (unsigned)std::min<size_t>((n + kBlock - 1) / kBlock, 2048);
    scale_kernel<<<g, kBlock, 0, st>>>(n, in, a, out);
    check_launch();
}

void copy(hipStream_t st, size_t n, const double* src, double* dst) {
    if (n && src != dst) PMC_HIP(hipMemcpyAsync(dst, src, n * sizeof(double), hipMemcpyDeviceToDevice, st));
}

void minres_init(hipStream_t st, int nb, MinresState* s, const DotParts& d, double rel_tol, double abs_tol, int ring) {
    minres_init_kernel<<<1, kScalBlock, 0, st>>>(s, d.p1, d.n1, nb, rel_tol, abs_tol, d.p2, d.n2, ring);
    check_launch();
}
void minres_scal1(hipStream_t st, int nb, MinresState* s, const DotParts& d) {
    minres_scal1_kernel<<<1, kScalBlock, 0, st>>>(s, d.p1, d.n1, nb, d.p2, d.n2);
    check_launch();
}
void minres_scal2(hipStream_t st, int nb, MinresState* s, const DotParts& d) {
    minres_scal2_kernel<<<1, kScalBlock, 0, st>>>(s, d.p1, d.n1, nb, d.p2, d.n2);
    check_launch();
}
size_t scal_stage_doubles() { return (size_t)2 * kStageBlocks * kMaxBatch; }
void minres_scal21(hipStream_t st, int nb, MinresState* s, const DotParts& d2, const DotParts& d1, double* stage) {
    if (stage && d2.total() + d1.total() >= 8 * kStageBlocks) {
        stage_partials_kernel<<<kStageBlocks, 256, 0, st>>>(d2.p1, d2.n1, d2.p2, d2.n2, d1.p1, d1.n1, d1.p2, d1.n2, nb, stage);
        check_launch();
        minres_scal21_kernel<<<1, kScalBlock, 0, st>>>(s, stage, kStageBlocks, nullptr, 0,
                                                        stage + (size_t)kStageBlocks * nb, kStageBlocks, nullptr, 0, nb);
    } else {
        minres_scal21_kernel<<<1, kScalBlock, 0, st>>>(s, d2.p1, d2.n1, d2.p2, d2.n2, d1.p1, d1.n1, d1.p2, d1.n2, nb);
    }
    check_launch();
}

void normal_fill(hipStream_t st, int n, int nbatch, uint64_t seed, uint64_t first_id, uint32_t stream, double mean,
                 double sigma, double* out, uint64_t id_stride) {
    if (n == 0 || nbatch == 0) return;
    const int npair = (n + 1) / 2;
    dim3 g((unsigned)((npair + kBlock - 1) / kBlock), (unsigned)nbatch);
    normal_fill_kernel<<<g, kBlock, 0, st>>>(n, nbatch, seed, first_id, id_stride, stream, mean, sigma, out);
    check_launch();
}

void interleave(hipStream_t st, int nb, int n, const double* in, const double* w, double scale, double* out, const int* src) {
    PMC_DISPATCH_NB(nb, { interleave_kernel<NB><<<groups(grid_rows(n), nb), kBlock, 0, st>>>(n, in, w, scale, out, nb, src); });
    check_launch();
}

void deinterleave(hipStream_t st, int nb, int m, const double* in, const int* idx, const double* rowscale, bool do_exp,
                  double* out) {
    if (m == 0) return;
    PMC_DISPATCH_NB(nb, { deinterleave_kernel<NB><<<groups(grid_rows(m), nb), kBlock, 0, st>>>(m, in, idx, rowscale, do_exp ? 1 : 0, out, nb); });
    check_launch();
}

void broadcast(hipStream_t st, int nb, int n, const double* a, double* out) {
    PMC_DISPATCH_NB(nb, { broadcast_kernel<NB><<<groups(grid_rows(n), nb), kBlock, 0, st>>>(n, a, out, nb); });
    check_launch();
}

void darcy_coef(hipStream_t st, int nb, int n, const double* kfield, bool k_divides, double* coef) {
    PMC_DISPATCH_NB(nb, { darcy_coef_kernel<NB><<<groups(grid_rows(n), nb), kBlock, 0, st>>>(n, kfield, k_divides ? 1 : 0, coef, nb); });
// ... 179 lines not shown
```

parelagmc_amd/csrc/kernels.hpp:

```cpp
#pragma once
#include "common.hpp"

namespace pmc {

struct zvec {
    void* p = nullptr;
    bool f32 = true;
    zvec() = default;
    zvec(void* p_, bool f32_) : p(p_), f32(f32_) {}
    size_t elem_bytes() const { return f32 ? 4 : 8; }
    zvec operator+(size_t elems) const { return zvec(static_cast<char*>(p) + elems * elem_bytes(), f32); }
    explicit operator bool() const { return p != nullptr; }
    template <typename T>
    T* as() const { return static_cast<T*>(p); }
};
inline zvec zconst(const double* p) { return zvec(const_cast<double*>(p), false); }
inline zvec zconst(const float* p) { return zvec(const_cast<float*>(p), true); }
struct ZBuf {
    DevBuf<float> b;
    void ensure(size_t count, bool f32) { b.ensure(f32 ? count : 2 * count); }
    zvec v(bool f32) const { return zvec(b.p, f32); }
};

struct SellView {
    int nrows = 0, nslices = 0;
    const int* slice_off = nullptr;
    const int* cols = nullptr;
    const double* vals = nullptr;
    bool bv = false;
    const int* sched = nullptr;
    int tag = 0;
    int ncols_hint = 0;
    bool diag_last = false;
    bool f32 = false;
    int split_log2 = 0;
};
inline SellView view(const Sell& S) {
    return {S.nrows, S.nslices, S.slice_off.p, S.cols.p, S.vals.p, false, S.sched.p, 0, S.ncols, S.diag_last};
}
inline SellView view_split(const Sell& S, int sl) {
    SellView v = view(S);
    v.split_log2 = sl;
    return v;
}
inline SellView view_bv(const Sell& S, const double* vals) {
    return {S.nrows, S.nslices, S.slice_off.p, S.cols.p, vals, true, S.sched.p, 0, S.ncols};
}
inline SellView view_bv32(const Sell& S, const float* vals) {
    SellView v = view_bv(S, reinterpret_cast<const double*>(vals));
    v.f32 = true;
    return v;
}

struct EgView {
    int nrows = 0, nslices = 0, gw = 0;
    const int* cols = nullptr;
    const double* w = nullptr;
    const int* e12 = nullptr;
};

int dot_capacity(int nrows, int nb);
uint64_t kernel_launch_count();
void count_kernel_launches(int n);

namespace k {

#ifndef PMC_WX_DEFER_N
#define PMC_WX_DEFER_N 8
#endif
static constexpr int kWxDefer = PMC_WX_DEFER_N;
static constexpr int kWxWindow = 32;
struct WxDeferred {
    const void* u[kWxWindow];
    int slot[kWxWindow];
    int cnt;
    bool f32;
    bool first;
    bool x_zero;
    bool last;
};

struct MinresState {
    double beta[kMaxBatch], beta_old[kMaxBatch], eta[kMaxBatch], eta0[kMaxBatch];
    double gamma0[kMaxBatch], gamma1[kMaxBatch], sigma0[kMaxBatch], sigma1[kMaxBatch];
    double goal[kMaxBatch], alpha[kMaxBatch], delta[kMaxBatch], rho2[kMaxBatch], rho3[kMaxBatch];
    double cV[3][kMaxBatch];
    int active[kMaxBatch], iters[kMaxBatch], flag[kMaxBatch];
    int n_active, it, ring;
    double cW[kWxWindow][4][kMaxBatch];
};
static constexpr size_t kMinresHeadBytes = offsetof(MinresState, cW);

int spmm(hipStream_t st, int nb, const SellView& A, const double* x, double* y, bool accumulate,
          double* dot_partial, const double* dot_with);
int spmm_z(hipStream_t st, int nb, const SellView& A, zvec x, double* y, double* dot_partial, zvec dot_with);
struct LanczosUpdate {
    const double* __restrict__ c0 = nullptr;
    const double* __restrict__ c1 = nullptr;
    const double* __restrict__ c2 = nullptr;
    const double* __restrict__ v1 = nullptr;
    float* __restrict__ y32 = nullptr;
};
int spmm_z_dot(hipStream_t st, int nb, const SellView& A, zvec x, double* dot_partial);
void spmm_z_update(hipStream_t st, int nb, const SellView& A, zvec x, const LanczosUpdate& lz, double* v, bool v_zero);
void residual_restrict8(hipStream_t st, int nb, const SellView& A, const double* r, const double* x, double* out,
                        double* coarse);
void residual(hipStream_t st, int nb, const SellView& A, const double* r, const double* x, double* out);
int cheb_step(hipStream_t st, int nb, const SellView& A, const double* dinv, bool dinv_bv, const double* r,
              const double* xin, double* d, double* xout, double a, double b, double* dot_partial = nullptr);
int cheb_step_z(hipStream_t st, int nb, const SellView& A, const double* dinv, bool dinv_bv, const double* r,
                const double* xin, double* d, zvec zout, double a, double b, double* dot_partial = nullptr);
int poly2(hipStream_t st, int nb, const SellView& As, const double* dinv, bool dinv_bv, const double* r, double* xout,
          double c0, double c1, double* dot_partial = nullptr, const double* xadd = nullptr,
          const double* dot_with = nullptr, const int* padd_idx = nullptr, const double* padd_x = nullptr);
int poly2_z(hipStream_t st, int nb, const SellView& As, const double* dinv, bool dinv_bv, const double* r, zvec xout,
            double c0, double c1, double* dot_partial = nullptr, const double* xadd = nullptr,
            const double* dot_with = nullptr, const int* padd_idx = nullptr, const double* padd_x = nullptr);
void vc_presmooth32(hipStream_t st, int nb, const SellView& As, const double* dinv, zvec r, float* xout, double c0, double c1);
void vc_residual_restrict8_32(hipStream_t st, int nb, const SellView& A, zvec r, const float* x, float* out, zvec coarse);
void vc_residual32(hipStream_t st, int nb, const SellView& A, zvec r, const float* x, float* out);
void vc_residual_restrict_agg32(hipStream_t st, int nb, const SellView& A, zvec r, const float* x, float* out, zvec coarse,
                                const int* seg_ptr, const int* seg_cid, const int* seg_pos);
void vc_restrict32(hipStream_t st, int nb, const SellView& Pt, const float* res, zvec coarse);
void vc_residual_coarse32(hipStream_t st, int nb, const SellView& SP, float* res, zvec xc);
int vc_postsmooth32_z(hipStream_t st, int nb, const SellView& As, const double* dinv, const float* res, const float* x,
                      zvec xout, double c0, double c1, const double* r, const int* parent, zvec xc, double* dot_partial);
void vc_presmooth32_bv(hipStream_t st, int nb, const SellView& As, const double* dinv, const double* r, float* xout, double c0,
                       double c1);
void vc_restrict8_32_bv(hipStream_t st, int nb, const SellView& A, const double* r, const float* x, double* coarse);
void vc_prolong8_32(hipStream_t st, int nb, int n, float* x, const double* xc);
void vc_residual32_bv(hipStream_t st, int nb, const SellView& A, const double* r, const float* x, float* out);
int vc_postsmooth32_bv(hipStream_t st, int nb, const SellView& As, const double* dinv, const float* res, const float* x,
                       double* xout, double c0, double c1, const double* r, double* dot_partial);
int vc_postsmooth32_bv_z(hipStream_t st, int nb, const SellView& As, const double* dinv, const float* res, const float* x,
                         zvec xout, double c0, double c1, const double* r, double* dot_partial);
int pair_spmm_z(hipStream_t st, int nb, const SellView& A1, zvec x1, const SellView& A2, zvec x2, double* y,
                double* dot_partial, zvec dot_with);
void scale_cols_bv(hipStream_t st, int nb, int64_t nslots, const int* cols, const double* vals, const double* colscale,
                   double* out);
void scale_cols_bv32(hipStream_t st, int nb, int64_t nslots, const int* cols, const double* vals, const double* colscale,
                     float* out_scaled, float* out_vals);
void minres_wx_idx(hipStream_t st, int nb, int nsel, const int* rows, const double* c0, zvec u, const double* c1,
                   double* w0, const double* c2, const double* w1, const double* c3, double* x);
int cheb_first(hipStream_t st, int nb, int n, const double* dinv, bool dinv_bv, const double* r, double* d,
               double* x, double b, double* dot_partial = nullptr);
int wdot(hipStream_t st, int nb, int n, const double* w, const double* x, double* partial);
int dot_z(hipStream_t st, int nb, int n, const double* a, zvec b, double* partial);
int convert_z(hipStream_t st, int nb, int n, const double* in, zvec out, const double* r, double* dot_partial);
void copy_r32(hipStream_t st, int nb, int n, const double* in, double* out, float* out32);
void reduce_final(hipStream_t st, int nb, int nblocks, const double* partial, double* out);
void lincomb3(hipStream_t st, int nb, int n, const double* c0, const double* a, const double* c1, const double* b,
              const double* c2, double* y, float* y32 = nullptr);
void minres_wx(hipStream_t st, int nb, int n, const double* c0, zvec u, const double* c1, double* w0,
               const double* c2, const double* w1, const double* c3, double* x);
void fill(hipStream_t st, size_t n, double* x, double v);
void copy(hipStream_t st, size_t n, const double* src, double* dst);
void scale(hipStream_t st, size_t n, const double* in, double a, double* out);

struct DotParts {
    const double* p1 = nullptr;
    int n1 = 0;
    const double* p2 = nullptr;
    int n2 = 0;
    int total() const { return n1 + n2; }
};
void minres_init(hipStream_t st, int nb, MinresState* s, const DotParts& d, double rel_tol, double abs_tol, int ring = 1);
void minres_wx_deferred(hipStream_t st, int nb, int n, const MinresState* s, const WxDeferred& B, double* w0, double* w1,
                        double* x);
void minres_scal1(hipStream_t st, int nb, MinresState* s, const DotParts& d);
void minres_scal2(hipStream_t st, int nb, MinresState* s, const DotParts& d);
void minres_scal21(hipStream_t st, int nb, MinresState* s, const DotParts& d2, const DotParts& d1, double* stage = nullptr);
size_t scal_stage_doubles();

void normal_fill(hipStream_t st, int n, int nbatch, uint64_t seed, uint64_t first_id, uint32_t stream, double mean,
                 double sigma, double* out, uint64_t id_stride = 1);
void interleave(hipStream_t st, int nb, int n, const double* in, const double* w, double scale, double* out,
                const int* src = nullptr);
void deinterleave(hipStream_t st, int nb, int m, const double* in, const int* idx, const double* rowscale, bool do_exp,
                  double* out);
void broadcast(hipStream_t st, int nb, int n, const double* a, double* out);

void darcy_coef(hipStream_t st, int nb, int n, const double* kfield, bool k_divides, double* coef);
void darcy_assemble(hipStream_t st, int nb, const SellView& Mp, const int* slot_src, const int* c_ptr, const int* c_elem,
                    const double* c_val, const double* coef, const unsigned char* ess, const double* ess_data,
                    const double* rhs0, double* mvals, double* diag, double* l1inv, double* rhs_bc);
int eg_pair_spmm(hipStream_t st, int nb, const EgView& M, const double* coef, const double* x1, const SellView& A2,
                 const double* x2, double* y, double* dot_partial, const double* dot_with);
int eg_pair_spmm_z(hipStream_t st, int nb, const EgView& M, const double* coef, zvec x1, const SellView& A2,
                   zvec x2, double* y, double* dot_partial, zvec dot_with);
int eg_poly2(hipStream_t st, int nb, const EgView& M, const double* coef, const double* dinv, const double* r, double* xout,
// ... 68 lines not shown
```

parelagmc_amd/csrc/sampler.hip:

```cpp
#include <algorithm>
#include <cmath>

#include <cstdlib>
#include <cstring>

#include "handles.hpp"

namespace pmc {

static bool diag_last_on() {
    static const bool v = [] {
        const char* e = lab_env("PMC_DIAG_LAST");
        return !e || atoi(e) != 0;
    }();
    return v;
}


HostCsr schur_host(const HostCsr& B, const HostCsr& Bt, const std::vector<double>& dM, const double* diag_add) {
    HostCsr S;
    S.nrows = S.ncols = B.nrows;
    S.rowptr.assign(B.nrows + 1, 0);
    std::vector<int> marker(B.nrows, -1);
    std::vector<std::pair<int, double>> row;
    for (int e = 0; e < B.nrows; ++e) {
        row.clear();
        auto add = [&](int c, double v) {
            if (marker[c] < 0) { marker[c] = (int)row.size(); row.emplace_back(c, v); }
            else row[marker[c]].second += v;
        };
        add(e, diag_add ? diag_add[e] : 0.0);
        for (int p = B.rowptr[e]; p < B.rowptr[e + 1]; ++p) {
            const int f = B.colind[p];
            const double w = B.vals[p] / dM[f];
            for (int q = Bt.rowptr[f]; q < Bt.rowptr[f + 1]; ++q) add(Bt.colind[q], w * Bt.vals[q]);
        }
        std::sort(row.begin(), row.end(), [](const auto& a, const auto& b) { return a.first < b.first; });
        for (auto& cv : row) { S.colind.push_back(cv.first); S.vals.push_back(cv.second); marker[cv.first] = -1; }
        S.rowptr[e + 1] = (int)S.colind.size();
    }
    return S;
}

struct AggSegments {
    std::vector<int> ptr, cid, pos;
};
bool spd_dense_inverse(const HostCsr& S, std::vector<double>& inv) {
    const int n = S.nrows;
    std::vector<double> a((size_t)n * n, 0.0);
    inv.assign((size_t)n * n, 0.0);
    for (int i = 0; i < n; ++i)
        for (int p = S.rowptr[i]; p < S.rowptr[i + 1]; ++p) a[(size_t)i * n + S.colind[p]] = S.vals[p];
    for (int j = 0; j < n; ++j) {
        double dj = a[(size_t)j * n + j];
        for (int k = 0; k < j; ++k) dj -= a[(size_t)j * n + k] * a[(size_t)j * n + k];
        if (!(dj > 0.0) || !std::isfinite(dj)) return false;
        const double l = std::sqrt(dj);
        a[(size_t)j * n + j] = l;
        for (int i = j + 1; i < n; ++i) {
            double v = a[(size_t)i * n + j];
            for (int k = 0; k < j; ++k) v -= a[(size_t)i * n + k] * a[(size_t)j * n + k];
            a[(size_t)i * n + j] = v / l;
        }
    }
    std::vector<double> y(n);
    for (int c = 0; c < n; ++c) {
        for (int i = 0; i < c; ++i) y[i] = 0.0;
        for (int i = c; i < n; ++i) {
            double v = i == c ? 1.0 : 0.0;
            for (int k = c; k < i; ++k) v -= a[(size_t)i * n + k] * y[k];
            y[i] = v / a[(size_t)i * n + i];
        }
        for (int i = n - 1; i >= 0; --i) {
            double v = y[i];
            for (int k = i + 1; k < n; ++k) v -= a[(size_t)k * n + i] * inv[(size_t)k * n + c];
            inv[(size_t)i * n + c] = v / a[(size_t)i * n + i];
        }
    }
    for (int i = 0; i < n; ++i)
        for (int j = 0; j < i; ++j) {
            const double v = 0.5 * (inv[(size_t)i * n + j] + inv[(size_t)j * n + i]);
            inv[(size_t)i * n + j] = inv[(size_t)j * n + i] = v;
// ... 338 lines not shown
        PMC_HIP(hipStreamSynchronize(st));
        if (getenv("PMC_VERBOSE")) {
            const Multigrid& h = *amg[l];
            fprintf(stderr, "[pmc] hybrid sampler level %d: n_lambda %d n_s %d nnz(H) %lld | V-cycle levels", l, d.n_u, d.n_s,
                    (long long)d.nnz);
            for (size_t q = 0; q < h.L.size(); ++q)
                fprintf(stderr, " %d%s%s", h.L[q].n, h.L[q].has_sp ? "i" : "", (q < h.tail.size() && h.tail[q].p) ? "t" : "");
            fprintf(stderr, "\n");
            for (size_t q = 0; q < h.L.size(); ++q)
                fprintf(stderr, "[pmc]   V-cycle level %zu: S %lld entries in %lld slots, S P %lld in %lld, lmax %.3f\n", q,
                        (long long)h.L[q].S.nnz, (long long)h.L[q].S.nslots, (long long)h.L[q].SP.nnz, (long long)h.L[q].SP.nslots,
                        h.L[q].lmax);
        }
    }
}

void Sampler::set_projection(int level, int kind, const pmc_csr* Gt, const int32_t* idx, const double* inv_w,
                             int orig_size) {
    PMC_REQUIRE(level >= 0 && level < n_mc, "set_projection: level out of range");
    PMC_REQUIRE(cond == nullptr, "set_projection: a conditioner is attached (pmc_sampler_set_conditioner); detach it first");
    SamplerLevel& d = lv[level];
    ctx.activate();
    hipStream_t st = ctx.stream;
    if (kind == PMC_PROJ_NONE) {
        d.proj = PMC_PROJ_NONE;
        d.out_size = d.n_s;
    } else if (kind == PMC_PROJ_GATHER) {
        PMC_REQUIRE(idx != nullptr && orig_size > 0 && orig_size <= d.n_s, "set_projection: bad gather arguments");
        for (int i = 0; i < orig_size; ++i) PMC_REQUIRE(idx[i] >= 0 && idx[i] < d.n_s, "set_projection: gather index out of range");
        d.gather.upload(idx, orig_size, st);
        d.proj = kind;
        d.out_size = orig_size;
    } else if (kind == PMC_PROJ_L2) {
        PMC_REQUIRE(Gt != nullptr && inv_w != nullptr, "set_projection: Gt / inv_w is NULL");
        HostCsr G = csr_from_c(*Gt, true, "Gt");
        PMC_REQUIRE(G.ncols == d.n_s && G.nrows == orig_size && orig_size > 0, "set_projection: Gt has the wrong shape");
        sell_build(d.Gt, G, true, false, st);
        d.inv_w.upload(inv_w, orig_size, st);
        d.proj = kind;
        d.out_size = orig_size;
    } else {
        throw Error(PMC_ERR_INVALID, "set_projection: unknown kind");
    }
    PMC_HIP(hipStreamSynchronize(st));
}

void Sampler::ensure(int level, int nb) {
    size_t nmax = 0, smax = 0;
    for (int l = 0; l <= level; ++l) {
        nmax = std::max(nmax, (size_t)lv[l].n_u + lv[l].n_s);
        smax = std::max(smax, (size_t)lv[l].n_s);
    }
    for (int l = level; l < nlevels; ++l) smax = std::max(smax, (size_t)lv[l].n_s);
    for (int l = 0; l < n_mc; ++l) smax = std::max(smax, (size_t)lv[l].out_size);
    rhs.ensure(nmax * nb);
    sol.ensure(nmax * nb);
    tA.ensure(smax * nb);
    tB.ensure(smax * nb);
    if (!hybrid) {
        cx.ensure((size_t)lv[level].n_u * nb);
        cd.ensure((size_t)lv[level].n_u * nb);
    }
    stage_in.ensure(smax * nb);
    stage_out.ensure(smax * nb);
    stage_emb.ensure(smax * nb);
}

void Sampler::sample(int level, uint64_t first_id, int nbatch, double* xi, int memspace) {
    PMC_REQUIRE(level >= 0 && level < n_mc, "Sample: level out of range");
    PMC_REQUIRE(nbatch >= 1 && xi != nullptr, "Sample: bad arguments");
    ctx.activate();
    hipStream_t st = ctx.stream;
    const int n = lv[level].n_s;
    if (memspace == PMC_MEM_DEVICE) {
        k::normal_fill(st, n, nbatch, ctx.seed, ctx.stream_id(first_id), (uint32_t)level, 0.0, 1.0, xi, (uint64_t)ctx.nparts);
    } else {
        DevBuf<double> tmp((size_t)n * nbatch);
        k::normal_fill(st, n, nbatch, ctx.seed, ctx.stream_id(first_id), (uint32_t)level, 0.0, 1.0, tmp.p, (uint64_t)ctx.nparts);
        PMC_HIP(hipMemcpyAsync(xi, tmp.p, sizeof(double) * n * nbatch, hipMemcpyDeviceToHost, st));
        PMC_HIP(hipStreamSynchronize(st));
    }
}

void Sampler::eval_chunk(int level, int xi_level, int nb, const double* xi_d, double* s_d, const double* init_d,
                         int init_level, bool use_init, double* emb_d, pmc_stats* stats) {
    hipStream_t st = ctx.stream;
    SamplerLevel& d = lv[level];
    const int n_u = d.n_u, n_s = d.n_s;
    ensure(level, nb);
    if (stats) ctx.phase_mark(0);
    if (hybrid) {
        double* fz = rhs.p + (size_t)n_u * nb;
        if (xi_level == level) {
            k::interleave(st, nb, n_s, xi_d, d.zw_sqrt.p, -g, fz);
        } else {
            double* cur = tA.p;
            double* nxt = tB.p;
            k::interleave(st, nb, lv[xi_level].n_s, xi_d, lv[xi_level].w_sqrt.p, -g, cur);
            for (int l = xi_level; l < level; ++l) {
                const bool final_step = l + 1 == level;
                k::spmm(st, nb, final_step ? view(d.Ptz) : view(mg.L[l].Pt), cur, final_step ? fz : nxt, false, nullptr, nullptr);
                std::swap(cur, nxt);
            }
        }
        k::spmm(st, nb, view(d.Gz), fz, rhs.p, false, nullptr, nullptr);
        if (stats) ctx.phase_mark(1);
        solve_system(level, nb, true, 0, n_u, stats);
        double* field = sol.p + (size_t)n_u * nb;
        k::residual(st, nb, view(d.Gl), fz, sol.p, field);
    } else {
    k::fill(st, (size_t)n_u * nb, rhs.p, 0.0);
    double* rhs_s = rhs.p + (size_t)n_u * nb;
    if (xi_level == level) {
        k::interleave(st, nb, n_s, xi_d, lv[xi_level].w_sqrt.p, -g, rhs_s);
    } else {
        double* cur = tA.p;
        double* nxt = tB.p;
        k::interleave(st, nb, lv[xi_level].n_s, xi_d, lv[xi_level].w_sqrt.p, -g, cur);
        for (int l = xi_level; l < level; ++l) {
            double* dst = (l + 1 == level) ? rhs_s : nxt;
            k::spmm(st, nb, view(mg.L[l].Pt), cur, dst, false, nullptr, nullptr);
            std::swap(cur, nxt);
        }
    }
    bool zero_guess = true;
    if (use_init) {
        double* sol_s = sol.p + (size_t)n_u * nb;
        k::fill(st, (size_t)n_u * nb, sol.p, 0.0);
        if (init_level == level) {
            k::interleave(st, nb, n_s, init_d, nullptr, 1.0, sol_s);
        } else {
            double* cur = tA.p;
            double* nxt = tB.p;
            k::interleave(st, nb, lv[init_level].n_s, init_d, nullptr, 1.0, cur);
            for (int l = init_level; l > level; --l) {
                double* dst = (l - 1 == level) ? sol_s : nxt;
                k::spmm(st, nb, view(mg.L[l - 1].P), cur, dst, false, nullptr, nullptr);
                std::swap(cur, nxt);
            }
        }
        zero_guess = false;
    }
    if (stats) ctx.phase_mark(1);
    solve_system(level, nb, zero_guess, n_u, n_s, stats);
    }
    const double* sol_s = sol.p + (size_t)n_u * nb;
    if (d.proj == PMC_PROJ_NONE) {
        k::deinterleave(st, nb, n_s, sol_s, nullptr, nullptr, lognormal && !cond, s_d);
        if (cond) cond->apply_device(level, nb, s_d, nullptr, s_d, lognormal);
    } else if (d.proj == PMC_PROJ_GATHER) {
        k::deinterleave(st, nb, d.out_size, sol_s, d.gather.p, nullptr, lognormal, s_d);
    } else {
        k::spmm(st, nb, view(d.Gt), sol_s, tA.p, false, nullptr, nullptr);
        k::deinterleave(st, nb, d.out_size, tA.p, nullptr, d.inv_w.p, lognormal, s_d);
    }
    if (emb_d) k::deinterleave(st, nb, n_s, sol_s, nullptr, nullptr, false, emb_d);
}

void Sampler::solve_system(int level, int nb, bool zero_guess, int x_row0, int x_nrows, pmc_stats* stats) {
    hipStream_t st = ctx.stream;
    SamplerLevel& d = lv[level];
    const int n_u = d.n_u, n_s = d.n_s, n = (int)system_rows(level);
    const bool use_amg = level < (int)amg.size() && amg[level];
    Multigrid* mgp = use_amg ? amg[level].get() : &mg;
    const int mg_l0 = use_amg ? 0 : level;
    static const int mini_env = [] {
        const char* e = lab_env("PMC_MINI_MAX_ROWS");
        return e ? atoi(e) : -1;
    }();
    const int mini_max_rows = mini_env >= 0 ? mini_env : opts.mini_max_rows;
    const int degM = opts.cheb_degree_M > 0 ? opts.cheb_degree_M : (d.ratio_M > 16.0 ? 4 : 2);
    const bool mini = !hybrid && n <= mini_max_rows && degM == 2 && opts.use_graph == 0 && mgp->use_tail &&
                      mg_l0 < (int)mgp->tail.size() && mgp->tail[mg_l0].p != nullptr;
    if (mini) {
        MiniSamplerParams mp{};
        mp.n_u = n_u;
        mp.n_s = n_s;
        mp.a_off = d.A.slice_off.p; mp.a_cols = d.A.cols.p; mp.a_vals = d.A.vals.p;
        mp.m_off = d.M.slice_off.p; mp.m_cols = d.M.cols.p; mp.m_scaled = d.M_scaled.p; mp.m_dinv = d.dinvM.p;
        cheb2_coefficients(1.0, d.ratio_M, &mp.mc0, &mp.mc1);
        mp.tail = mgp->tail[mg_l0].p;
        mp.max_iter = opts.max_iter;
        mp.rel_tol = opts.rel_tol;
        mp.abs_tol = opts.abs_tol;
        mp.x_row0 = x_row0;
        mp.x_nrows = x_nrows;
        mp.scratch_per_col = (size_t)5 * n + (size_t)3 * x_nrows;
        mini_scratch.ensure(mp.scratch_per_col * nb);
        mini_stats.ensure(kMaxBatch);
        k::mini_sampler_solve(st, nb, mp, mgp->tail_lds[mg_l0], rhs.p, sol.p, zero_guess, mini_scratch.p, mini_stats.p);
        if (stats) {
            ctx.phase_mark(2);
            PMC_HIP(hipMemcpyAsync(ctx.h_scal, mini_stats.p, sizeof(pmc_stats) * nb, hipMemcpyDeviceToHost, st));
            PMC_HIP(hipStreamSynchronize(st));
            std::memcpy(stats, ctx.h_scal, sizeof(pmc_stats) * nb);
            ctx.phase_report(stats, nb);
        }
    } else {
    LinOp A;
    A.n = n;
    A.n0 = hybrid ? 0 : n_u;
    SellView Av = view(d.A);
    Av.tag = 1;
    A.apply = [Av](const Lanes& L, int nb_, const double* x, double* y, double* partial, double*) {
        return k::DotParts{partial, k::spmm(L.main, nb_, Av, x, y, false, partial, x)};
    };
    A.apply_z = [Av](const Lanes& L, int nb_, zvec x, double* y, double* partial, double*) {
        return k::DotParts{partial, k::spmm_z(L.main, nb_, Av, x, y, partial, x)};
    };
    if (hybrid && !Av.bv) {
        A.apply_z_dot = [Av](const Lanes& L, int nb_, zvec x, double* partial, double*) {
            return k::DotParts{partial, k::spmm_z_dot(L.main, nb_, Av, x, partial)};
        };
        A.apply_z_update = [Av](const Lanes& L, int nb_, zvec x, const k::LanczosUpdate& lz, double* v, bool v_zero) {
            k::spmm_z_update(L.main, nb_, Av, x, lz, v, v_zero);
        };
    }
    PrecFn prec = preconditioner(level, nb, degM, mgp, mg_l0);
    work.want_r32 = hybrid && opts.precond_storage != PMC_STORAGE_FP64 && mgp->top_reads_r32(mg_l0, nb);
    if (const char* e = lab_env("PMC_R32")) work.want_r32 = work.want_r32 && atoi(e) != 0;
    work.r32_valid = false;
    mgp->smooth_timer = (hybrid && work.op_timer.on && opts.use_graph == 0) ? &vc_timer : nullptr;
    vc_timer.on = mgp->smooth_timer != nullptr;
    GraphHint hint;
    hint.key = hash_mix(hash_mix(hash_mix(0x5a, (uint64_t)level + 1), (uint64_t)nb), (uint64_t)x_row0);
    hint.sig = hash_ptr(hash_ptr(hash_ptr(mgp->signature(mg_l0), cx.p), cd.p), cx2.p);
    MinresResult res = minres_solve(ctx, nb, A, prec, rhs.p, sol.p, zero_guess, opts, work, x_row0, x_nrows, nullptr, hint);
    if (vc_timer.on) vc_timer.harvest();
    if (stats) {
        ctx.phase_mark(2);
        for (int kcol = 0; kcol < nb; ++kcol) stats[kcol] = res.col[kcol];
        ctx.phase_report(stats, nb);
    }
    }
}

PrecFn Sampler::preconditioner(int level, int nb, int degM, Multigrid* mgp, int mg_l0) {
    SamplerLevel& d = lv[level];
    const int n_u = d.n_u;
    if (hybrid) {
        (void)nb; (void)degM;
        return [=](const Lanes& L, int nb_, const double* r, zvec z, double* dot_partial, double*) {
            mgp->r32_top = work.r32_valid ? work.r32.p : nullptr;
            work.r32_valid = false;
            const int nblk = mgp->vcycle_z(L.main, nb_, mg_l0, r, z, dot_partial);
            return k::DotParts{dot_partial, nblk, nullptr, 0};
        };
    }
    const SellView Mv = view(d.M);
    const double* dinvM = d.dinvM.p;
    ChebParams cpM{degM, 1.0, d.ratio_M, d.M_scaled.p};
    if (!cheb_fused(cpM, true)) cx2.ensure((size_t)n_u * nb);
    double* cxp = cx.p;
    double* cx2p = cx2.p;
    double* cdp = cd.p;
    return [=](const Lanes& L, int nb_, const double* r, zvec z, double* dot_partial, double* dot_partial2) {
        int nblk_u = 0;
        auto m_block = [&]() {
            L.fork();
            nblk_u = cheb_apply_z(L.side(), nb_, Mv, dinvM, false, cpM, r, z, cxp, cx2p, cdp, dot_partial2);
        };
        const int nblk_s = mgp->vcycle_z(L.main, nb_, mg_l0, r + (size_t)n_u * nb_, z + (size_t)n_u * nb_, dot_partial, m_block);
        L.join();
        return k::DotParts{dot_partial, nblk_s, dot_partial2, nblk_u};
    };
}

double Sampler::smoother_bytes(int level, int nb) const {
    if (!hybrid || level < 0 || level >= n_mc || !amg[level] || amg[level]->L.size() < 2) return 0.0;
    const MgLevel& m = amg[level]->L[0];
    const double zb = opts.precond_storage == PMC_STORAGE_FP64 ? 8.0 : 4.0;
    const double cb = amg[level]->inner_f32(1, 0, nb) ? 4.0 : 8.0;
    return 12.0 * (double)m.S.nnz + 12.0 * m.n + (double)nb * ((4.0 + 4.0 + 8.0 + zb) * m.n + cb * amg[level]->L[1].n);
}

void Sampler::apply_preconditioner(int level, int nbatch, const double* r_in, double* z_out, int memspace) {
    PMC_REQUIRE(level >= 0 && level < n_mc, "apply_preconditioner: level out of range");
    PMC_REQUIRE(valid_batch(nbatch) && nbatch <= batch_width((size_t)lv[level].n_u + lv[level].n_s, false, ctx.device) && r_in != nullptr && z_out != nullptr,
                "apply_preconditioner: nbatch must be a launch width of the level");
    ctx.activate();
    hipStream_t st = ctx.stream;
    SamplerLevel& d = lv[level];
    const size_t n = system_rows(level);
    const int nb = nbatch;
    ensure(level, nb);
    DevBuf<double> stage, zi(n * nb), part((size_t)2 * dot_capacity((int)n, nb) * nb);
    const double* r_d = r_in;
    if (memspace == PMC_MEM_HOST) {
        stage.alloc(n * nb);
        PMC_HIP(hipMemcpyAsync(stage.p, r_in, sizeof(double) * n * nb, hipMemcpyHostToDevice, st));
        r_d = stage.p;
    }
    k::interleave(st, nb, (int)n, r_d, nullptr, 1.0, rhs.p, hybrid ? d.lam_new2old.p : nullptr);
    const bool use_amg = level < (int)amg.size() && amg[level];
    Multigrid* mgp = use_amg ? amg[level].get() : &mg;
    const int degM = opts.cheb_degree_M > 0 ? opts.cheb_degree_M : (d.ratio_M > 16.0 ? 4 : 2);
    PrecFn prec = preconditioner(level, nb, degM, mgp, use_amg ? 0 : level);
    prec(ctx.lanes(false), nb, rhs.p, zvec(zi.p, false), part.p, part.p + (size_t)dot_capacity((int)n, nb) * nb);
    double* out_d = memspace == PMC_MEM_HOST ? stage.p : z_out;
    k::deinterleave(st, nb, (int)n, zi.p, hybrid ? d.lam_old2new.p : nullptr, nullptr, false, out_d);
    if (memspace == PMC_MEM_HOST) PMC_HIP(hipMemcpyAsync(z_out, stage.p, sizeof(double) * n * nb, hipMemcpyDeviceToHost, st));
    PMC_HIP(hipStreamSynchronize(st));
}

void Sampler::mult(int level, int nbatch, const double* rhs_in, double* sol_io, bool use_guess, int memspace, pmc_stats* stats) {
    PMC_REQUIRE(level >= 0 && level < n_mc, "Mult: level out of range");
    PMC_REQUIRE(nbatch >= 1 && rhs_in != nullptr && sol_io != nullptr, "Mult: bad arguments");
    ctx.activate();
    hipStream_t st = ctx.stream;
    const size_t n = system_rows(level);
// ... 188 lines not shown
```

parelagmc_amd/csrc/solver.hip:

```cpp
#include "solver.hpp"

#include <atomic>
#include <cmath>
#include <cstddef>
#include <cstdlib>
#include <cstring>

namespace pmc {

double* cheb_apply(hipStream_t st, int nb, const SellView& A, const double* dinv, bool dinv_bv, const ChebParams& cp,
                   const double* r, double* xa, double* xb, double* d, bool zero_guess, double* dot_partial,
                   int* dot_blocks, zvec zlast) {
    if (cp.degree < 1) throw Error(PMC_ERR_INVALID, "Chebyshev degree must be >= 1");
    const double lmax = cp.lmax, lmin = cp.lmax / cp.ratio;
    const double theta = 0.5 * (lmax + lmin), delta = 0.5 * (lmax - lmin);
    const double sigma = theta / delta;
    double rho_old = 1.0 / sigma;
    if (cheb_fused(cp, zero_guess)) {
        const double rho1 = 1.0 / (2.0 * sigma - rho_old);
        const double c0 = (1.0 + rho1 * rho_old) / theta + 2.0 * rho1 / delta;
        const double c1 = 2.0 * rho1 / (delta * theta);
        SellView As = A;
        As.vals = cp.scaled_vals;
        int nblk;
// ... 419 lines not shown
static bool stage_on() {
    static const bool v = [] {
        const char* e = lab_env("PMC_SCAL_STAGE");
        return !e || atoi(e) != 0;
    }();
    return v;
}
static size_t sampler_wide_rows(int device) {
    static std::atomic<size_t> cache[64];
    const int slot = device & 63;
    size_t v = cache[slot].load(std::memory_order_relaxed);
    if (v == 0) {
        size_t total_b = 0;
        hipDevice_t dev;
        if (hipDeviceGet(&dev, device) != hipSuccess || hipDeviceTotalMem(&total_b, dev) != hipSuccess || total_b == 0)
            v = (size_t)5000000;
        else
            v = (size_t)((double)total_b * 0.5 / (110.0 * 32.0 * 8.0));
        cache[slot].store(v, std::memory_order_relaxed);
    }
    return v;
}

static size_t wx_ring_budget(int device) {
    static std::atomic<size_t> cache[64];
    const int slot = device & 63;
    size_t v = cache[slot].load(std::memory_order_relaxed);
    if (v == 0) {
        size_t total_b = 0;
        hipDevice_t dev;
        if (hipDeviceGet(&dev, device) != hipSuccess || hipDeviceTotalMem(&total_b, dev) != hipSuccess) total_b = 0;
        v = total_b / 128 + 1;
        cache[slot].store(v, std::memory_order_relaxed);
    }
    return v - 1;
}

int batch_width(size_t rows, bool darcy, int device) {
    static const auto lim = [](const char* name, size_t dflt) {
        const char* e = lab_env(name);
        return e ? (size_t)atoll(e) : dflt;
    };
    static const size_t l32 = lim("PMC_WIDE_ROWS", 300000),
                        l32s_lab = lim("PMC_S_WIDE_ROWS", lab_env("PMC_WIDE_ROWS") ? l32 : 0),
                        l64 = lim("PMC_W64_ROWS", 150000), l128 = lim("PMC_W128_ROWS", 40000), l256 = lim("PMC_W256_ROWS", 20000),
                        l64s = lim("PMC_S_W64_ROWS", lab_env("PMC_W64_ROWS") ? l64 : 700000);
    const size_t l32s = l32s_lab ? l32s_lab : (darcy ? 0 : sampler_wide_rows(device));
    if (rows > (darcy ? l32 : l32s)) return 16;
    if (rows <= l256) return 256;
    if (rows <= l128) return 128;
    if (rows <= (darcy ? l64 : l64s)) return 64;
    return 32;
}

static bool wx_defer_on() {
    static const bool v = [] {
        const char* e = lab_env("PMC_WX_DEFER");
        return !e || atoi(e) != 0;
    }();
    return v;
}

static int wx_window(int device, size_t vec_bytes) {
    static const int lab = [] {
        const char* e = lab_env("PMC_WX_WINDOW");
        return e ? std::min(std::max(atoi(e), 1), k::kWxWindow) : 0;
    }();
    if (lab) return lab;
    const size_t fit = wx_ring_budget(device) / std::max<size_t>(vec_bytes, 1);
    return (int)std::min<size_t>(std::max<size_t>(fit, 9) - 1, (size_t)k::kWxWindow);
}

static std::atomic<uint64_t> g_fused_solves{0};
uint64_t fused_lanczos_solve_count() { return g_fused_solves.load(std::memory_order_relaxed); }

static bool fused_lanczos_on() {
    static const bool v = [] {
        const char* e = lab_env("PMC_FUSED_LANCZOS");
        return !e || atoi(e) != 0;
    }();
    return v;
}

static bool late_wx() {
    static const bool v = [] {
        const char* e = lab_env("PMC_LATE_WX");
        return !e || atoi(e) != 0;
    }();
    return v;
}

MinresResult minres_solve(Ctx& ctx, int nb, const LinOp& A, const PrecFn& prec, const double* b, double* x,
                          bool zero_guess, const pmc_solver_opts& o, MinresWork& w, int x_row0, int x_nrows,
                          const int* x_rows, GraphHint hint) {
    hipStream_t st = ctx.stream;
    const int n = A.n;
    const size_t len = (size_t)n * nb;
    const bool split = o.two_streams == 1 || (o.two_streams == 0 && split_threshold() > 0 && len >= split_threshold() &&
                                              Ctx::contexts_on_device(ctx.device) == 1);
    const Lanes L = ctx.lanes(split);
    const bool z32 = o.precond_storage != PMC_STORAGE_FP64;
    const int every = o.check_every > 0 ? o.check_every : 1;
    const bool graphs = hint.key != 0 && o.use_graph != 0 && every == 2;
    const bool late = L.split && !graphs && A.n0 > 0 && A.n0 < n && late_wx();
    const bool r32 = w.want_r32 && z32;
    const bool timing = w.op_timer.on && !(hint.key != 0 && o.use_graph != 0);
    const bool fused = A.apply_z_dot && A.apply_z_update && !graphs && !late && r32 && !timing && fused_lanczos_on();
    w.ensure(n, nb, z32, !fused);
    if (r32) w.r32.ensure(len);
    k::MinresState* S = w.state.p;
    double* v0 = w.v0.p; double* v1 = w.v1.p; zvec u0 = w.u0.v(z32); zvec u1 = w.u1.v(z32);
    double* w0 = w.w0.p; double* w1 = w.w1.p; double* q = w.q.p;

    if (x_rows && !zero_guess) throw Error(PMC_ERR_INTERNAL, "minres: compact solution needs a zero initial guess");
    if (!A.apply_z || (!zero_guess && !A.apply)) throw Error(PMC_ERR_INTERNAL, "minres: operator closures missing");
    if (x_row0 < 0 || x_nrows < 0 || (!x_rows && x_row0 + x_nrows > n))
        throw Error(PMC_ERR_INTERNAL, "minres: bad solution row range");
    if (fused) g_fused_solves.fetch_add(1, std::memory_order_relaxed);
    const size_t xoff = (size_t)x_row0 * nb;
    const bool defer = !graphs && !late && !x_rows && wx_defer_on();
    if (zero_guess) {
        if (defer) {
            k::fill(st, xoff, x, 0.0);
            k::fill(st, len - xoff - (size_t)x_nrows * nb, x + xoff + (size_t)x_nrows * nb, 0.0);
        } else {
            k::fill(st, x_rows ? (size_t)x_nrows * nb : len, x, 0.0);
        }
        if (r32) k::copy_r32(st, nb, n, b, v1, w.r32.p);
        else k::copy(st, len, b, v1);
    } else {
        A.apply(L, nb, x, v1, nullptr, nullptr);
        axpby(st, len, 1.0, b, -1.0, v1);
        if (r32) k::convert_z(st, nb, n, v1, zvec(reinterpret_cast<double*>(w.r32.p), true), nullptr, nullptr);
    }
    const size_t seg2 = (size_t)dot_capacity(n, nb) * nb;
    w.r32_valid = r32;
    k::DotParts dp = prec(L, nb, v1, u1, w.partial.p, w.partial.p + seg2);
    if (dp.total() == 0) dp = k::DotParts{w.partial.p, k::dot_z(st, nb, n, v1, u1, w.partial.p)};
    const int window = defer ? wx_window(ctx.device, len * (z32 ? sizeof(float) : sizeof(double))) : 1;
    k::minres_init(st, nb, S, dp, o.rel_tol, o.abs_tol, window);
    if (!fused) k::fill(st, len, v0, 0.0);
    if (!defer) {
        k::fill(st, len, w0, 0.0);
        k::fill(st, len, w1, 0.0);
    }

    auto coef = [&](size_t off) { return reinterpret_cast<const double*>(reinterpret_cast<const char*>(S) + off); };
    const double* cV0 = coef(offsetof(k::MinresState, cV));
    const double* cV1 = cV0 + kMaxBatch;
    const double* cV2 = cV1 + kMaxBatch;
    const double* cW0 = coef(offsetof(k::MinresState, cW));
    const double* cW1 = cW0 + kMaxBatch;
    const double* cW2 = cW1 + kMaxBatch;
    const double* cW3 = cW2 + kMaxBatch;
    const int* d_nactive = reinterpret_cast<const int*>(reinterpret_cast<const char*>(S) + offsetof(k::MinresState, n_active));

    auto poll = [&]() {
        PMC_HIP(hipMemcpyAsync(ctx.h_flag, d_nactive, sizeof(int), hipMemcpyDeviceToHost, st));
        PMC_HIP(hipStreamSynchronize(st));
        return *ctx.h_flag;
    };

    MinresResult out;
    zvec u2;
    if (late) {
        w.u2.ensure(len, z32);
        u2 = w.u2.v(z32);
    }
    k::DotParts dp_op;
    auto apply_op = [&](zvec u) {
        if (fused) {
            dp_op = A.apply_z_dot(L, nb, u, w.partial_op.p, w.partial_op.p + seg2);
            return;
        }
        if (timing) w.op_timer.begin(st);
        dp_op = A.apply_z(L, nb, u, q, w.partial_op.p, w.partial_op.p + seg2);
        if (timing) w.op_timer.end(st);
    };
    struct PendingWx { zvec u; double *w0 = nullptr, *w1 = nullptr; } pend;
    auto wx = [&](hipStream_t s, zvec u_, double* w0_, double* w1_) {
        if (x_rows) k::minres_wx_idx(s, nb, x_nrows, x_rows, cW0, u_, cW1, w0_, cW2, w1_, cW3, x);
        else k::minres_wx(s, nb, x_nrows, cW0, u_ + xoff, cW1, w0_, cW2, w1_, cW3, x + xoff);
    };
    auto flush_wx = [&](hipStream_t s) {
        if (pend.u) wx(s, pend.u, pend.w0, pend.w1);
        pend.u = zvec();
    };
    int it = 0;
    auto iteration = [&](zvec u0_, zvec u1_, double* v0_, double* v1_, double* w0_, double* w1_, bool last) {
        if (fused) {
            k::LanczosUpdate lz;
            lz.c0 = cV0; lz.c1 = cV1; lz.c2 = cV2;
            lz.v1 = v1_;
            lz.y32 = w.r32.p;
            A.apply_z_update(L, nb, u1_, lz, v0_, it == 1);
            w.r32_valid = true;
        } else if (late) {
            const size_t off = (size_t)A.n0 * nb;
            L.fork();
            k::lincomb3(L.aux, nb, A.n0, cV0, q, cV1, v1_, cV2, v0_);
            flush_wx(L.aux);
            k::lincomb3(st, nb, n - A.n0, cV0, q + off, cV1, v1_ + off, cV2, v0_ + off);
        } else {
            k::lincomb3(st, nb, n, cV0, q, cV1, v1_, cV2, v0_, r32 ? w.r32.p : nullptr);
            w.r32_valid = r32;
        }
        k::DotParts d2 = prec(L, nb, v0_, u0_, w.partial.p, w.partial.p + seg2);
        if (d2.total() == 0) d2 = k::DotParts{w.partial.p, k::dot_z(st, nb, n, v0_, u0_, w.partial.p)};
        if (!last) {
            apply_op(u0_);
            k::minres_scal21(st, nb, S, d2, dp_op, stage_on() ? w.stage.p : nullptr);
// ... 161 lines not shown
```

parelagmc_amd/csrc/solver.hpp:

```cpp
#pragma once
#include <functional>
#include <map>
#include <vector>

#include "kernels.hpp"

namespace pmc {

struct ChebParams {
    int degree = 3;
    double lmax = 1.0;
    double ratio = 8.0;
    const double* scaled_vals = nullptr;
};
inline void cheb2_coefficients(double lmax, double ratio, double* c0, double* c1) {
    const double lmin = lmax / ratio;
    const double theta = 0.5 * (lmax + lmin), delta = 0.5 * (lmax - lmin), sigma = theta / delta;
    const double rho_old = 1.0 / sigma, rho1 = 1.0 / (2.0 * sigma - rho_old);
    *c0 = (1.0 + rho1 * rho_old) / theta + 2.0 * rho1 / delta;
    *c1 = 2.0 * rho1 / (delta * theta);
}
inline bool cheb_fused(const ChebParams& cp, bool ) { return cp.degree == 2 && cp.scaled_vals; }
double* cheb_apply(hipStream_t st, int nb, const SellView& A, const double* dinv, bool dinv_bv, const ChebParams& cp,
                   const double* r, double* xa, double* xb, double* d, bool zero_guess,
// ... 21 lines not shown
    double lmax = 2.0;
    bool is_last = false;
    int last_degree = 12;
    double last_ratio = 100.0;
    Sell P, Pt;
    HostCsr P_host;
    Sell SP;
    DevBuf<int> parent;
    bool has_sp = false;
    bool p_oct = false;
    bool p_agg = false;
    DevBuf<int> seg_ptr, seg_cid, seg_pos;
    DevBuf<double> r, xa, xb, d, res;
    DevBuf<double> ainv;
    DevBuf<double> dense_inv;
    int split_log2 = 0, sp_split_log2 = 0;
    Sell S_split, SP_split;
    DevBuf<double> scaled_split;
    void ensure(int nb);
    SellView sview() const { return bv ? (f32 ? view_bv32(S, vals32.p) : view_bv(S, vals_bv.p)) : view(S); }
    const double* scaled_ptr() const { return (bv && f32) ? reinterpret_cast<const double*>(scaled32.p) : vals_scaled.p; }
};

struct OpTimer;
struct Multigrid {
    std::vector<MgLevel> L;
    int smooth_degree = 2;
    double smooth_ratio = 4.0;
    int coarse_degree = 12;
    double coarse_ratio = 100.0;
    std::vector<DevBuf<TailParams>> tail;
    std::vector<size_t> tail_lds;
    bool use_tail = true;
    bool f32_intermediates = true;
    bool f32_any_injection = false;
    int tail_later_nb = 0;
    int dense_nb = 0;
    const float* r32_top = nullptr;
    bool top_reads_r32(int l0, int nb) const {
        if (l0 < 0 || l0 + 1 >= (int)L.size()) return false;
        const MgLevel& lv = L[(size_t)l0];
        const bool tail_later = nb <= tail_later_nb && lv.n > 4096 && l0 + 1 < (int)tail.size() && tail[(size_t)l0 + 1].p;
        const bool tail_here = use_tail && l0 < (int)tail.size() && tail[(size_t)l0].p && !tail_later;
        return !tail_here && !lv.is_last && !lv.bv && lv.has_sp && !lv.p_oct && f32_any_injection && smooth_degree == 2 &&
               lv.vals_scaled.p && f32_intermediates;
    }
    OpTimer* smooth_timer = nullptr;
    void build_tails(hipStream_t st);
    void enable_bv_tail(int max_rows = 8192);
    int bv_tail_width = 0;
    void ensure_bv_tail_width(hipStream_t st, int nb);
    void refresh_bv_tail(hipStream_t st, int nb, int first_level = 0);
    int cycle_role(int l0, int nb, int l, bool* in_tail) const;
    uint64_t signature(int l0) const;
    int vcycle(hipStream_t st, int nb, int l0, const double* r, double* xout, double* dot_partial = nullptr,
               const std::function<void()>& side = nullptr);
    int vcycle_z(hipStream_t st, int nb, int l0, const double* r, zvec zout, double* dot_partial = nullptr,
                 const std::function<void()>& side = nullptr);

    struct LevelPath {
        bool last = false, dense = false, tail_here = false, f32_shared = false, f32_bv = false;
    };
    LevelPath level_path(int l, int l0, int nb) const;
    bool inner_f32(int l, int l0, int nb) const;

  private:
    zvec cycle(hipStream_t st, int nb, int l, int l0, zvec rz, double* target, zvec ztarget, double* dot_partial,
               int* dot_blocks, const std::function<void()>* side);
};

struct LinOp {
    int n = 0;
    int n0 = 0;
    std::function<k::DotParts(const Lanes& L, int nb, const double* x, double* y, double* dot_partial,
                              double* dot_partial2)> apply;
    std::function<k::DotParts(const Lanes& L, int nb, zvec x, double* y, double* dot_partial,
                              double* dot_partial2)> apply_z;
    std::function<k::DotParts(const Lanes& L, int nb, zvec x, double* dot_partial, double* dot_partial2)> apply_z_dot;
    std::function<void(const Lanes& L, int nb, zvec x, const k::LanczosUpdate& lz, double* v, bool v_zero)> apply_z_update;
};
using PrecFn = std::function<k::DotParts(const Lanes& L, int nb, const double* r, zvec z, double* dot_partial,
                                         double* dot_partial2)>;

struct GraphHint {
    uint64_t key = 0, sig = 0;
};
inline uint64_t hash_mix(uint64_t h, uint64_t v) {
    h ^= v + 0x9E3779B97F4A7C15ull + (h << 6) + (h >> 2);
    return h;
}
inline uint64_t hash_ptr(uint64_t h, const void* p) { return hash_mix(h, (uint64_t)(uintptr_t)p); }

struct OpTimer {
    bool on = false;
    std::vector<hipEvent_t> ev;
    size_t used = 0;
    double ms = 0.0, gap_ms = 0.0;
    int64_t launches = 0;
    OpTimer() = default;
    OpTimer(const OpTimer&) = delete;
    OpTimer& operator=(const OpTimer&) = delete;
    ~OpTimer() {
        for (hipEvent_t e : ev) (void)hipEventDestroy(e);
    }
    void begin(hipStream_t st) {
        while (ev.size() < used + 3) {
            hipEvent_t e;
            PMC_HIP(hipEventCreate(&e));
            ev.push_back(e);
        }
        PMC_HIP(hipEventRecord(ev[used], st));
    }
    void end(hipStream_t st) {
        PMC_HIP(hipEventRecord(ev[used + 1], st));
        PMC_HIP(hipEventRecord(ev[used + 2], st));
        used += 3;
    }
    void harvest() {
        for (size_t e = 0; e + 2 < used; e += 3) {
            float a = 0.f, g = 0.f;
            PMC_HIP(hipEventElapsedTime(&a, ev[e], ev[e + 1]));
            PMC_HIP(hipEventElapsedTime(&g, ev[e + 1], ev[e + 2]));
            ms += a;
            gap_ms += g;
            ++launches;
        }
        used = 0;
    }
    void clear() { ms = gap_ms = 0.0; launches = 0; }
};

struct MinresWork {
    DevBuf<double> v0, v1, w0, w1, q, partial;
    ZBuf u0, u1;
    DevBuf<double> stage;
    ZBuf u2;
    std::vector<ZBuf> ring;
    DevBuf<double> partial_op;
    DevBuf<float> r32;
    bool want_r32 = false, r32_valid = false;
    std::map<uint64_t, int> iter_hint;
    DevBuf<k::MinresState> state;
    struct GraphEntry {
        uint64_t sig = 0;
        hipGraphExec_t exec = nullptr;
    };
    std::map<uint64_t, GraphEntry> graphs;
    OpTimer op_timer;
    MinresWork() = default;
    MinresWork(const MinresWork&) = delete;
    MinresWork& operator=(const MinresWork&) = delete;
    ~MinresWork();
    void ensure(int n, int nb, bool z32, bool need_q = true);
};

uint64_t fused_lanczos_solve_count();

struct MinresResult {
    pmc_stats col[kMaxBatch];
    int iterations = 0;
};

MinresResult minres_solve(Ctx& ctx, int nb, const LinOp& A, const PrecFn& prec, const double* b, double* x,
                          bool zero_guess, const pmc_solver_opts& o, MinresWork& w, int x_row0, int x_nrows,
                          const int* x_rows = nullptr, GraphHint hint = GraphHint());

double gershgorin_scaled(const HostCsr& A, const std::vector<double>& diag, double* lmin = nullptr);

}
```

Baseline: 4245 samples/s.

## Fuse RHS construction into MINRES start and field residual with exp and de-interleave

The right-hand side G_z*f is now produced inside the MINRES setup. The SpMV writes both the fp64 Lanczos vector and its fp32 copy directly, which removes a separate rhs buffer write and the copy_r32 pass. The final field evaluation fuses the Gl residual, the optional lognormal exp and the sample-major output layout into one kernel, skipping the intermediate field buffer and later transforms when there is no projection, conditioning or embedding. The deferred w/x update kernel also processes several rows per thread to reuse the coefficient loads. Together these add complexity, including an adopt path that only applies without graphs or split lanes.

Measured after the change: 4354 samples/s (median of 6 runs). 2.6% higher.

```diff
diff --git a/include/pmc.h b/include/pmc.h
--- a/include/pmc.h
+++ b/include/pmc.h
@@ -109,6 +109,8 @@
 int pmc_darcy_krylov_z_bytes(const pmc_darcy* d);
 uint64_t pmc_kernel_launches(void);
 uint64_t pmc_fused_lanczos_solves(void);
+uint64_t pmc_adopted_rhs_solves(void);
+uint64_t pmc_fused_field_evals(void);
 const char* pmc_last_error(void);
 void pmc_solver_opts_default(pmc_solver_opts* opts);
 
diff --git a/parelagmc_amd/capi.py b/parelagmc_amd/capi.py
--- a/parelagmc_amd/capi.py
+++ b/parelagmc_amd/capi.py
@@ -92,6 +92,8 @@
     "pmc_darcy_krylov_z_bytes": (C.c_int, [_VP]),
     "pmc_kernel_launches": (C.c_uint64, []),
     "pmc_fused_lanczos_solves": (C.c_uint64, []),
+    "pmc_adopted_rhs_solves": (C.c_uint64, []),
+    "pmc_fused_field_evals": (C.c_uint64, []),
     "pmc_ctx_create": (C.c_int, [C.c_int, C.POINTER(_VP)]),
     "pmc_ctx_create_abi": (C.c_int, [C.c_int, C.c_int, C.POINTER(_VP)]),
     "pmc_ctx_destroy": (None, [_VP]),
@@ -213,6 +215,8 @@
     "pmc_allreduce_sum_f64": (C.c_int, [_VP, C.POINTER(C.c_double), C.c_int]),
 }
 
+_LATE_DIAGNOSTICS = ("pmc_adopted_rhs_solves", "pmc_fused_field_evals")
+
 _lib = None
 
 
@@ -225,6 +229,8 @@
         raise PmcError(-2, f"{p} not found - build it with `make` / __graft_entry__.build() (no CPU fallback)")
     lib = C.CDLL(p)
     for name, (res, args) in SYMBOLS.items():
+        if name in _LATE_DIAGNOSTICS and not hasattr(lib, name):
+            continue
         fn = getattr(lib, name)
         fn.restype = res
         fn.argtypes = args
diff --git a/parelagmc_amd/csrc/capi.hip b/parelagmc_amd/csrc/capi.hip
--- a/parelagmc_amd/csrc/capi.hip
+++ b/parelagmc_amd/csrc/capi.hip
@@ -104,6 +104,8 @@
 int pmc_krylov_z_bytes(void) { return 4; }
 uint64_t pmc_kernel_launches(void) { return kernel_launch_count(); }
 uint64_t pmc_fused_lanczos_solves(void) { return fused_lanczos_solve_count(); }
+uint64_t pmc_adopted_rhs_solves(void) { return adopted_rhs_solve_count(); }
+uint64_t pmc_fused_field_evals(void) { return fused_field_eval_count(); }
 const char* pmc_last_error(void) { return g_last_error.c_str(); }
 
 static void check_abi(const pmc_solver_opts& o) {
diff --git a/parelagmc_amd/csrc/handles.hpp b/parelagmc_amd/csrc/handles.hpp
--- a/parelagmc_amd/csrc/handles.hpp
+++ b/parelagmc_amd/csrc/handles.hpp
@@ -33,6 +33,8 @@
     DevBuf<int> lam_new2old, lam_old2new;
     std::vector<int> lam_n2o_host;
 };
+
+uint64_t fused_field_eval_count();
 
 struct Sampler {
     Ctx& ctx;
@@ -89,7 +91,7 @@
 
   private:
     void ensure(int level, int nb);
-    void solve_system(int level, int nb, bool zero_guess, int x_row0, int x_nrows, pmc_stats* stats);
+    void solve_system(int level, int nb, bool zero_guess, int x_row0, int x_nrows, pmc_stats* stats, const RhsFn* rhs = nullptr);
     PrecFn preconditioner(int level, int nb, int degM, Multigrid* mgp, int mg_l0);
     void eval_chunk(int level, int xi_level, int nb, const double* xi_d, double* s_d, const double* init_d,
                     int init_level, bool use_init, double* emb_d, pmc_stats* stats);
diff --git a/parelagmc_amd/csrc/kernels.hip b/parelagmc_amd/csrc/kernels.hip
--- a/parelagmc_amd/csrc/kernels.hip
+++ b/parelagmc_amd/csrc/kernels.hip
@@ -26,7 +26,7 @@
 }
 
 template <int NB, int BV, int MODE, bool DOT, int TAG, bool NT = false, bool R8 = false, bool DL = false, typename XT = double,
-          typename YT = double, int LZ = 0>
+          typename YT = double, int LZ = 0, int SM = 0>
 __global__ __launch_bounds__(kBlock, (NB >= 32 && BV == 0 && sizeof(XT) == 4 ? 3 : 1)) void sell_spmm_kernel(int nrows, int nslices, const int* __restrict__ slice_off,
                                                            const int* __restrict__ sched,
                                                            const int* __restrict__ cols,
@@ -40,19 +40,23 @@
     static_assert(LZ == 0 || (BV == 0 && MODE == 0 && !R8 && sizeof(YT) == 8 && DOT == (LZ == 1)),
                   "Lanczos passes: shared values, plain product; the dot-only pass has the dot, the update passes none");
     static_assert(sizeof(YT) == 8 || (MODE == 0 && !DOT && !NT), "fp32 result: plain products only");
+    static_assert(SM == 0 || (MODE == 2 && BV == 0 && !DOT && !R8 && LZ == 0 && sizeof(YT) == 8),
+                  "sample-major result: the plain residual of a shared-value matrix");
     const int LD = row_ld<NB>(ld);
     {
         const int c0 = col0<NB>();
         x += c0;
-        if constexpr (LZ != 1) y += c0;
+        if constexpr (SM) y += (size_t)c0 * nrows;
+        else if constexpr (LZ != 1) y += c0;
         if constexpr (BV) vals = shift_bv<BV>(vals, c0);
         if constexpr (MODE == 2) r += c0;
         if constexpr (DOT && !DL) dot_with += c0;
         if constexpr (DOT || R8) partial += c0;
-        if constexpr (LZ >= 2) {
-            lz.v1 += c0; lz.y32 += c0;
+        if constexpr (LZ == 2 || LZ == 3) {
+            lz.v1 += c0;
             lz.c0 += c0; lz.c1 += c0; lz.c2 += c0;
         }
+        if constexpr (LZ >= 2) lz.y32 += c0;
     }
     static_assert(!DL || (DOT && !BV && Lay<NB>::T > 1), "diagonal-last serves the fused <x, Ax> of shared-value operators");
     constexpr int C = Lay<NB>::C, T = Lay<NB>::T, G = Lay<NB>::G;
@@ -97,7 +101,17 @@
 #pragma unroll
                     for (int c = 0; c < C; ++c) acc[rs][c] = rv[c] - acc[rs][c];
                 }
-                if constexpr (LZ >= 2) {
+                if constexpr (LZ == 4) {
+                    store_c<C>(y + at, acc[rs]);
+                    store_v<C>(lz.y32 + at, acc[rs]);
+                } else if constexpr (SM) {
+#pragma unroll
+                    for (int c = 0; c < C; ++c) {
+                        double tv = acc[rs][c];
+                        if constexpr (SM == 2) tv = exp(tv);
+                        y[(size_t)(t * C + c) * nrows + row] = tv;
+                    }
+                } else if constexpr (LZ >= 2) {
                     double bv[C], yv[C];
                     load_c_nt<NT, C>(lz.v1 + at, bv);
                     if constexpr (LZ == 2) {
@@ -946,53 +960,82 @@
     }
 }
 
+template <typename UT, int C>
+struct WxShape {
+    static constexpr int R = sizeof(UT) == 4 ? 4 : 2;
+    static constexpr int Dfit = 64 / (R * C * (int)(sizeof(UT) / 4));
+    static constexpr int D = Dfit < 1 ? 1 : (Dfit > k::kWxDefer ? k::kWxDefer : Dfit);
+};
 template <int NB, bool NT, typename UT>
 __global__ __launch_bounds__(kBlock) void minres_wx_deferred_kernel(size_t nflat, k::WxDeferred B,
                                                                     const double* __restrict__ cW, double* __restrict__ w0,
                                                                     double* __restrict__ w1, double* __restrict__ x, int ld) {
     constexpr int C = Lay<NB>::C;
-    const size_t i = (size_t)blockIdx.x * kBlock + threadIdx.x;
-    if (i >= nflat) return;
-    const size_t e = i * C;
-    const int k0 = (int)(e % row_ld<NB>(ld));
-    double a[C], b[C], xv[C];
-    if (B.first) {
-#pragma unroll
-        for (int c = 0; c < C; ++c) a[c] = b[c] = 0.0;
-    } else {
-        load_c_nt<NT, C>(w0 + e, a);
-        load_c_nt<NT, C>(w1 + e, b);
-    }
-    if (B.first && B.x_zero) {
-#pragma unroll
-        for (int c = 0; c < C; ++c) xv[c] = 0.0;
-    } else {
-        load_c_nt<NT, C>(x + e, xv);
-    }
-    for (int t = 0; t < B.cnt; t += k::kWxDefer) {
-        RawVec<UT, C> uv[k::kWxDefer];
-#pragma unroll
-        for (int j = 0; j < k::kWxDefer; ++j)
-            if (t + j < B.cnt) load_raw_nt<NT>(static_cast<const UT*>(B.u[t + j]) + e, uv[j]);
-#pragma unroll
-        for (int j = 0; j < k::kWxDefer; ++j) {
+    constexpr int R = WxShape<UT, C>::R, D = WxShape<UT, C>::D;
+    const size_t i0 = (size_t)blockIdx.x * (R * kBlock) + threadIdx.x;
+    if (i0 >= nflat) return;
+    const int k0 = (int)((i0 * C) % row_ld<NB>(ld));
+    size_t e[R];
+    bool live[R];
+#pragma unroll
+    for (int r = 0; r < R; ++r) {
+        const size_t i = i0 + (size_t)r * kBlock;
+        live[r] = i < nflat;
+        e[r] = (live[r] ? i : i0) * C;
+    }
+    double a[R][C], b[R][C], xv[R][C];
+#pragma unroll
+    for (int r = 0; r < R; ++r) {
+        if (B.first) {
+#pragma unroll
+            for (int c = 0; c < C; ++c) a[r][c] = b[r][c] = 0.0;
+        } else {
+            load_c_nt<NT, C>(w0 + e[r], a[r]);
+            load_c_nt<NT, C>(w1 + e[r], b[r]);
+        }
+        if (B.first && B.x_zero) {
+#pragma unroll
+            for (int c = 0; c < C; ++c) xv[r][c] = 0.0;
+        } else {
+            load_c_nt<NT, C>(x + e[r], xv[r]);
+        }
+    }
+    for (int t = 0; t < B.cnt; t += D) {
+        RawVec<UT, C> uv[D][R];
+#pragma unroll
+        for (int j = 0; j < D; ++j) {
+            if (t + j < B.cnt) {
+                const UT* up = static_cast<const UT*>(B.u[t + j]);
+#pragma unroll
+                for (int r = 0; r < R; ++r) load_raw_nt<NT>(up + e[r], uv[j][r]);
+            }
+        }
+#pragma unroll
+        for (int j = 0; j < D; ++j) {
             if (t + j < B.cnt) {
                 const double* cj = cW + (size_t)B.slot[t + j] * 4 * kMaxBatch + k0;
 #pragma unroll
-                for (int c = 0; c < C; ++c) {
-                    const double wn = cj[c] * (double)uv[j].v[c] + cj[kMaxBatch + c] * a[c] + cj[2 * kMaxBatch + c] * b[c];
-                    xv[c] += cj[3 * kMaxBatch + c] * wn;
-                    a[c] = b[c];
-                    b[c] = wn;
+                for (int r = 0; r < R; ++r) {
+#pragma unroll
+                    for (int c = 0; c < C; ++c) {
+                        const double wn = cj[c] * (double)uv[j][r].v[c] + cj[kMaxBatch + c] * a[r][c] + cj[2 * kMaxBatch + c] * b[r][c];
+                        xv[r][c] += cj[3 * kMaxBatch + c] * wn;
+                        a[r][c] = b[r][c];
+                        b[r][c] = wn;
+                    }
                 }
             }
         }
     }
-    if (!B.last) {
-        store_c_nt<NT, C>(w0 + e, a);
-        store_c_nt<NT, C>(w1 + e, b);
-    }
-    store_c_nt<NT, C>(x + e, xv);
+#pragma unroll
+    for (int r = 0; r < R; ++r) {
+        if (!live[r]) continue;
+        if (!B.last) {
+            store_c_nt<NT, C>(w0 + e[r], a[r]);
+            store_c_nt<NT, C>(w1 + e[r], b[r]);
+        }
+        store_c_nt<NT, C>(x + e[r], xv[r]);
+    }
 }
 
 template <int NB>
@@ -1960,6 +2003,10 @@
 static inline dim3 grid_slices(int nslices) { return dim3((unsigned)((nslices + kBlock / kWave - 1) / (kBlock / kWave))); }
 static inline int lay_c(int nb) { return nb >= 32 ? 4 : (nb >= 2 ? 2 : 1); }
 static inline size_t flat_count(int n, int nb) { return (size_t)n * nb / lay_c(nb); }
+static inline unsigned wx_deferred_blocks(size_t nflat, int rows) {
+    const size_t per = (size_t)rows * kBlock;
+    return (unsigned)((nflat + per - 1) / per);
+}
 static inline dim3 grid_flat(int n, int nb) { return dim3((unsigned)((flat_count(n, nb) + kBlock - 1) / kBlock)); }
 static std::atomic<uint64_t> g_kernel_launches{0};
 uint64_t kernel_launch_count() { return g_kernel_launches.load(std::memory_order_relaxed); }
@@ -2157,6 +2204,33 @@
     check_launch();
 }
 
+void spmm_store32(hipStream_t st, int nb, const SellView& A, const double* x, double* y, float* y32) {
+    check_offsets32(A, nb);
+    if (A.bv || A.tag != 0 || !y || !y32) throw Error(PMC_ERR_INTERNAL, "spmm_store32: shared values, an untagged matrix, both results");
+    if (A.nrows == 0) return;
+    const dim3 g = grid_slices(A.nslices);
+    LanczosUpdate lz{};
+    lz.y32 = y32;
+    PMC_DISPATCH_NB(nb, {
+        sell_spmm_kernel<NB, false, 0, false, 0, false, false, false, double, double, 4><<<groups_xcd(g, nb), kBlock, 0, st>>>(A.nrows, A.nslices, A.slice_off, A.sched, A.cols, A.vals, x, y, nullptr, nullptr, nullptr, nb, lz);
+    });
+    check_launch();
+}
+
+void residual_samples(hipStream_t st, int nb, const SellView& A, const double* r, const double* x, bool do_exp, double* out) {
+    check_offsets32(A, nb);
+    if (A.bv) throw Error(PMC_ERR_INTERNAL, "residual_samples: shared values only");
+    if (A.nrows == 0) return;
+    const dim3 g = grid_slices(A.nslices);
+    PMC_DISPATCH_NB(nb, {
+        if (do_exp)
+            sell_spmm_kernel<NB, false, 2, false, 0, false, false, false, double, double, 0, 2><<<groups_xcd(g, nb), kBlock, 0, st>>>(A.nrows, A.nslices, A.slice_off, A.sched, A.cols, A.vals, x, out, r, nullptr, nullptr, nb);
+        else
+            sell_spmm_kernel<NB, false, 2, false, 0, false, false, false, double, double, 0, 1><<<groups_xcd(g, nb), kBlock, 0, st>>>(A.nrows, A.nslices, A.slice_off, A.sched, A.cols, A.vals, x, out, r, nullptr, nullptr, nb);
+    });
+    check_launch();
+}
+
 void residual(hipStream_t st, int nb, const SellView& A, const double* r, const double* x, double* out) {
     check_offsets32(A, nb);
     if (A.nrows == 0) return;
@@ -2736,13 +2810,17 @@
     if (B.cnt < 0 || B.cnt > kWxWindow) throw Error(PMC_ERR_INTERNAL, "minres_wx_deferred: bad count");
     const double* cW = reinterpret_cast<const double*>(reinterpret_cast<const char*>(s) + offsetof(MinresState, cW));
     const bool nt = nt_flat((size_t)n * nb);
+    if ((kBlock * lay_c(nb)) % nb != 0) throw Error(PMC_ERR_INTERNAL, "minres_wx_deferred: row stride does not divide a workgroup's step");
+    const size_t nf = flat_count(n, nb);
     PMC_DISPATCH_NB(nb, {
+        constexpr int C = Lay<NB>::C;
+        const dim3 g32(wx_deferred_blocks(nf, WxShape<float, C>::R)), g64(wx_deferred_blocks(nf, WxShape<double, C>::R));
         if (B.f32) {
-            if (nt) minres_wx_deferred_kernel<NB, true, float><<<grid_flat(n, nb), kBlock, 0, st>>>(flat_count(n, nb), B, cW, w0, w1, x, nb);
-            else minres_wx_deferred_kernel<NB, false, float><<<grid_flat(n, nb), kBlock, 0, st>>>(flat_count(n, nb), B, cW, w0, w1, x, nb);
+            if (nt) minres_wx_deferred_kernel<NB, true, float><<<g32, kBlock, 0, st>>>(nf, B, cW, w0, w1, x, nb);
+            else minres_wx_deferred_kernel<NB, false, float><<<g32, kBlock, 0, st>>>(nf, B, cW, w0, w1, x, nb);
         } else {
-            if (nt) minres_wx_deferred_kernel<NB, true, double><<<grid_flat(n, nb), kBlock, 0, st>>>(flat_count(n, nb), B, cW, w0, w1, x, nb);
-            else minres_wx_deferred_kernel<NB, false, double><<<grid_flat(n, nb), kBlock, 0, st>>>(flat_count(n, nb), B, cW, w0, w1, x, nb);
+            if (nt) minres_wx_deferred_kernel<NB, true, double><<<g64, kBlock, 0, st>>>(nf, B, cW, w0, w1, x, nb);
+            else minres_wx_deferred_kernel<NB, false, double><<<g64, kBlock, 0, st>>>(nf, B, cW, w0, w1, x, nb);
         }
     });
     check_launch();
diff --git a/parelagmc_amd/csrc/kernels.hpp b/parelagmc_amd/csrc/kernels.hpp
--- a/parelagmc_amd/csrc/kernels.hpp
+++ b/parelagmc_amd/csrc/kernels.hpp
@@ -106,6 +106,8 @@
 void residual_restrict8(hipStream_t st, int nb, const SellView& A, const double* r, const double* x, double* out,
                         double* coarse);
 void residual(hipStream_t st, int nb, const SellView& A, const double* r, const double* x, double* out);
+void residual_samples(hipStream_t st, int nb, const SellView& A, const double* r, const double* x, bool do_exp, double* out);
+void spmm_store32(hipStream_t st, int nb, const SellView& A, const double* x, double* y, float* y32);
 int cheb_step(hipStream_t st, int nb, const SellView& A, const double* dinv, bool dinv_bv, const double* r,
               const double* xin, double* d, double* xout, double a, double b, double* dot_partial = nullptr);
 int cheb_step_z(hipStream_t st, int nb, const SellView& A, const double* dinv, bool dinv_bv, const double* r,
diff --git a/parelagmc_amd/csrc/sampler.hip b/parelagmc_amd/csrc/sampler.hip
--- a/parelagmc_amd/csrc/sampler.hip
+++ b/parelagmc_amd/csrc/sampler.hip
@@ -1,3 +1,4 @@
+#include <atomic>
 #include <algorithm>
 #include <cmath>
 
@@ -502,6 +503,9 @@
     }
 }
 
+static std::atomic<uint64_t> g_fused_field_evals{0};
+uint64_t fused_field_eval_count() { return g_fused_field_evals.load(std::memory_order_relaxed); }
+
 void Sampler::eval_chunk(int level, int xi_level, int nb, const double* xi_d, double* s_d, const double* init_d,
                          int init_level, bool use_init, double* emb_d, pmc_stats* stats) {
     hipStream_t st = ctx.stream;
@@ -523,11 +527,23 @@
                 std::swap(cur, nxt);
             }
         }
-        k::spmm(st, nb, view(d.Gz), fz, rhs.p, false, nullptr, nullptr);
+        const SellView Gzv = view(d.Gz);
+        RhsFn make_rhs;
+        make_rhs.store = rhs.p;
+        make_rhs.write = [Gzv, fz](const Lanes& L, int nb_, double* y, float* y32) {
+            if (y32) k::spmm_store32(L.main, nb_, Gzv, fz, y, y32);
+            else k::spmm(L.main, nb_, Gzv, fz, y, false, nullptr, nullptr);
+        };
         if (stats) ctx.phase_mark(1);
-        solve_system(level, nb, true, 0, n_u, stats);
+        solve_system(level, nb, true, 0, n_u, stats, &make_rhs);
+        const SellView Glv = view(d.Gl);
+        if (d.proj == PMC_PROJ_NONE && !cond && !emb_d && !Glv.bv) {
+            k::residual_samples(st, nb, Glv, fz, sol.p, lognormal, s_d);
+            g_fused_field_evals.fetch_add(1, std::memory_order_relaxed);
+            return;
+        }
         double* field = sol.p + (size_t)n_u * nb;
-        k::residual(st, nb, view(d.Gl), fz, sol.p, field);
+        k::residual(st, nb, Glv, fz, sol.p, field);
     } else {
     k::fill(st, (size_t)n_u * nb, rhs.p, 0.0);
     double* rhs_s = rhs.p + (size_t)n_u * nb;
@@ -577,7 +593,7 @@
     if (emb_d) k::deinterleave(st, nb, n_s, sol_s, nullptr, nullptr, false, emb_d);
 }
 
-void Sampler::solve_system(int level, int nb, bool zero_guess, int x_row0, int x_nrows, pmc_stats* stats) {
+void Sampler::solve_system(int level, int nb, bool zero_guess, int x_row0, int x_nrows, pmc_stats* stats, const RhsFn* rhs_fn) {
     hipStream_t st = ctx.stream;
     SamplerLevel& d = lv[level];
     const int n_u = d.n_u, n_s = d.n_s, n = (int)system_rows(level);
@@ -645,7 +661,7 @@
     GraphHint hint;
     hint.key = hash_mix(hash_mix(hash_mix(0x5a, (uint64_t)level + 1), (uint64_t)nb), (uint64_t)x_row0);
     hint.sig = hash_ptr(hash_ptr(hash_ptr(mgp->signature(mg_l0), cx.p), cd.p), cx2.p);
-    MinresResult res = minres_solve(ctx, nb, A, prec, rhs.p, sol.p, zero_guess, opts, work, x_row0, x_nrows, nullptr, hint);
+    MinresResult res = minres_solve(ctx, nb, A, prec, rhs.p, sol.p, zero_guess, opts, work, x_row0, x_nrows, nullptr, hint, rhs_fn);
     if (vc_timer.on) vc_timer.harvest();
     if (stats) {
         ctx.phase_mark(2);
diff --git a/parelagmc_amd/csrc/solver.hip b/parelagmc_amd/csrc/solver.hip
--- a/parelagmc_amd/csrc/solver.hip
+++ b/parelagmc_amd/csrc/solver.hip
@@ -525,6 +525,9 @@
     return v;
 }
 
+static std::atomic<uint64_t> g_adopted_rhs_solves{0};
+uint64_t adopted_rhs_solve_count() { return g_adopted_rhs_solves.load(std::memory_order_relaxed); }
+
 static bool late_wx() {
     static const bool v = [] {
         const char* e = lab_env("PMC_LATE_WX");
@@ -535,7 +538,7 @@
 
 MinresResult minres_solve(Ctx& ctx, int nb, const LinOp& A, const PrecFn& prec, const double* b, double* x,
                           bool zero_guess, const pmc_solver_opts& o, MinresWork& w, int x_row0, int x_nrows,
-                          const int* x_rows, GraphHint hint) {
+                          const int* x_rows, GraphHint hint, const RhsFn* rhs) {
     hipStream_t st = ctx.stream;
     const int n = A.n;
     const size_t len = (size_t)n * nb;
@@ -559,7 +562,14 @@
     if (!A.apply_z || (!zero_guess && !A.apply)) throw Error(PMC_ERR_INTERNAL, "minres: operator closures missing");
     if (x_row0 < 0 || x_nrows < 0 || (!x_rows && x_row0 + x_nrows > n))
         throw Error(PMC_ERR_INTERNAL, "minres: bad solution row range");
+    if (rhs && (!rhs->write || !rhs->store)) throw Error(PMC_ERR_INTERNAL, "minres: right-hand side producer incomplete");
     if (fused) g_fused_solves.fetch_add(1, std::memory_order_relaxed);
+    const bool adopt = rhs && zero_guess && r32 && !graphs && !L.split;
+    if (rhs && !adopt) {
+        rhs->write(L, nb, rhs->store, nullptr);
+        b = rhs->store;
+    }
+    if (adopt) g_adopted_rhs_solves.fetch_add(1, std::memory_order_relaxed);
     const size_t xoff = (size_t)x_row0 * nb;
     const bool defer = !graphs && !late && !x_rows && wx_defer_on();
     if (zero_guess) {
@@ -569,7 +579,8 @@
         } else {
             k::fill(st, x_rows ? (size_t)x_nrows * nb : len, x, 0.0);
         }
-        if (r32) k::copy_r32(st, nb, n, b, v1, w.r32.p);
+        if (adopt) rhs->write(L, nb, v1, w.r32.p);
+        else if (r32) k::copy_r32(st, nb, n, b, v1, w.r32.p);
         else k::copy(st, len, b, v1);
     } else {
         A.apply(L, nb, x, v1, nullptr, nullptr);
diff --git a/parelagmc_amd/csrc/solver.hpp b/parelagmc_amd/csrc/solver.hpp
--- a/parelagmc_amd/csrc/solver.hpp
+++ b/parelagmc_amd/csrc/solver.hpp
@@ -127,6 +127,11 @@
 using PrecFn = std::function<k::DotParts(const Lanes& L, int nb, const double* r, zvec z, double* dot_partial,
                                          double* dot_partial2)>;
 
+struct RhsFn {
+    std::function<void(const Lanes& L, int nb, double* y, float* y32)> write;
+    double* store = nullptr;
+};
+
 struct GraphHint {
     uint64_t key = 0, sig = 0;
 };
@@ -200,6 +205,7 @@
 };
 
 uint64_t fused_lanczos_solve_count();
+uint64_t adopted_rhs_solve_count();
 
 struct MinresResult {
     pmc_stats col[kMaxBatch];
@@ -208,7 +214,7 @@
 
 MinresResult minres_solve(Ctx& ctx, int nb, const LinOp& A, const PrecFn& prec, const double* b, double* x,
                           bool zero_guess, const pmc_solver_opts& o, MinresWork& w, int x_row0, int x_nrows,
-                          const int* x_rows = nullptr, GraphHint hint = GraphHint());
+                          const int* x_rows = nullptr, GraphHint hint = GraphHint(), const RhsFn* rhs = nullptr);
 
 double gershgorin_scaled(const HostCsr& A, const std::vector<double>& diag, double* lmin = nullptr);
 
```
